# redmod-team/SympGPR

Measured on AMD Instinct MI355X. Metric: Gram-build GB/s + Cholesky fp64 TFLOP/s at N=65536 d=2; |alpha-alpha_ref|/|alpha_ref|, higher is better.
Workload: dtype f64

## Files before the change

### include/sympgpr_probe.h

```cpp
#ifndef SYMPGPR_PROBE_H
#define SYMPGPR_PROBE_H
#include <stddef.h>
#ifdef __cplusplus
extern "C" {
#endif

int sgpr_probe_mfma_f64(int waves_per_simd, int iters, double *tflops);
int sgpr_probe_hbm_write(size_t bytes, int reps, double *gbs);
int sgpr_probe_mfma_clock(int nacc, int waves_per_simd, int iters, double *out3);
int sgpr_probe_gemm(int m, int n, int k, int lower, double *out4);
int sgpr_probe_gemm_debug(int bits);
int sgpr_probe_leaf(double *out8);
int sgpr_probe_lat(double *out8);
int sgpr_probe_xcc(int nblocks, int *host_out);
int sgpr_probe_cumask(const unsigned *mask_words, int nwords, int nblocks, int *host_out);

int sgpr_probe_generated_eval(int family, int which, int m, const double *xa, const double *ya,
                              const double *xb, const double *yb, const double *l, int nl, double *out);

int sgpr_probe_queue_plan(int n, int nworkers, int *starts_out, int max_starts, unsigned *tasks_out, int max_tasks,
                          int *counts);
int sgpr_probe_queue_plan_partial(int n, int nworkers, int nq, int *starts_out, int max_starts, unsigned *tasks_out,
                                  int max_tasks, int *counts);
int sgpr_probe_queue_trace_begin(int max_tasks);
int sgpr_probe_queue_trace_end(unsigned long long *out, int max_tasks);
int sgpr_probe_queue_trace_clear(void);
int sgpr_probe_queue_postmortem(int always);
int sgpr_probe_queue_force_giveup(int on);
int sgpr_probe_tune(const char *name, double value);
int sgpr_probe_strassen_plan(int m, int n, int k, int lower, long smin, long kslab, long scratch_doubles, long long *out,
                             int max_records, int *count);
int sgpr_probe_gemm_strassen_dev(int m, int n, int k, double alpha, const double *A, size_t lda, const double *B, size_t ldb,
                                 double beta, double *C, size_t ldc, int lower, void *stream);
int sgpr_probe_gemm_nt2_dev(int m, int n, int k, double alpha, const double *A, size_t lda, const double *B, size_t ldb,
                            double beta, double *C, size_t ldc, double alpha2, double *C2, size_t ldc2, void *stream);
int sgpr_probe_strassen2_plan(int m, int n, int k, int lower, long smin, long kslab, long smin2, long kslab2, long scratch_doubles,
                              long long *out, int max_records, int *count);
int sgpr_probe_gemm_nt4_dev(int m, int n, int k, const double *A, size_t lda, const double *B, size_t ldb, double beta, int count,
                            double *const *C, const size_t *ldc, const double *alpha, void *stream);
int sgpr_probe_strassen_rec_plan(int m, int n, int k, int lower, long scratch_doubles, long cfg_out[5], long long *out,
                                 int max_records, int *count);
int sgpr_probe_strassen_rec_scratch(int n, unsigned long long out[2]);
int sgpr_probe_gemm_strassen_rec_dev(int m, int n, int k, double alpha, const double *A, size_t lda, const double *B, size_t ldb,
                                     double beta, double *C, size_t ldc, int lower, void *stream);
int sgpr_probe_strassen_schedule(int m, int n, int k, int lower, long capacity_doubles, long long info[12], long long *out,
                                 int max_records, int *count);
int sgpr_probe_batch_layout(int path, int mode, int d, int reg, int nbatch, int n_pts, int nhyp, unsigned long long out[24]);
int sgpr_probe_batch_layout_nd_loo(int path, int mode, int d, int nbatch, int n_pts, int nhyp, unsigned long long out[24]);
int sgpr_probe_batch_layout_loograd_mid(int d, int reg, int nbatch, int n_pts, int nhyp, unsigned long long out[32]);
unsigned sgpr_probe_map_calls(void);
int sgpr_probe_map_team(int ntest, int n0);

int sgpr_probe_trsm_piece(int ticket, int cap, int strips, int out[5]);
int sgpr_probe_trsm_counts(int strips, int cap, unsigned long long out[2]);

int sgpr_probe_census(int na, int threads_a, int lds_a, int spin_a, const unsigned *mask_a, int nwords_a,
                      int nb, int threads_b, int lds_b, int spin_b, const unsigned *mask_b, int nwords_b,
                      unsigned long long *host_out);

int sgpr_probe_strassen_top_plan(int m, int n, int k, int lower, long scratch_doubles, long long *out, int max_records, int *count);
int sgpr_probe_strassen_cfg_plan(int m, int n, int k, int lower, const long cfg[5], long long *out, int max_records, int *count);
int sgpr_probe_strassen_top_scratch(int n, unsigned long long out[2]);
int sgpr_probe_gemm_strassen_top_dev(int m, int n, int k, double alpha, const double *A, size_t lda, const double *B, size_t ldb,
                                     double beta, double *C, size_t ldc, int lower, void *stream);

#ifdef __cplusplus
}
#endif
#endif
```

### sympgpr_amd/_lib.py

```python
import ctypes as C
import os

import numpy as np

FAMILIES = {"A": 0, "B": 1, "C": 2, "D": 3, "USER": 4}
K_KERN, K_DXDX0, K_DYDY0, K_DXDY0 = 0, 1, 2, 3
K_DLX, K_DLY = 4, 8
K_DX, K_DY, K_DX0, K_DY0, K_DXDX0DY0, K_DYDY0DY0, K_DXDY0DY0 = 16, 17, 18, 19, 20, 21, 22
G_QQ, G_PQ, G_QP, G_PP, G_ALL, G_LOWER, G_OCML, G_DLX, G_DLY = 1, 2, 4, 8, 15, 16, 32, 64, 128
FIT_LOWER_ONLY, FIT_REG, FIT_BLOCK_QQ, FIT_BLOCK_PP = 1, 4, 8, 16
MAP_WRAP_Q, MAP_WRAP_P, MAP_EXPLICIT, MAP_LOSS_NEGP = 1, 2, 4, 8
E_ARG, E_NODEVICE, E_HIP, E_NOMEM, E_STATE = -1, -2, -3, -4, -5
LOO_LPD, LOO_PRESS = 0, 1

ABI_VERSION = 5
_dp = C.POINTER(C.c_double)
_vp = C.c_void_p


class SympGPRError(RuntimeError):
    code = None
    detail = ""


class NoDeviceError(SympGPRError):
    pass


def lib_path():
    return os.path.join(os.path.dirname(os.path.abspath(__file__)), "lib", "libsympgpr_hip.so")


SIGNATURES = {
    "sgpr_abi_version": (C.c_int, []),
    "sgpr_last_error": (C.c_char_p, []),
    "sgpr_device_count": (C.c_int, []),
    "sgpr_set_device": (C.c_int, [C.c_int]),
    "sgpr_build_k_host": (C.c_int, [C.c_int, C.c_int, C.c_int, _dp, _dp, _dp, _dp, _dp, C.c_int, _dp, C.c_size_t]),
    "sgpr_buildkreg_host": (C.c_int, [C.c_int, C.c_int, C.c_int, _dp, _dp, _dp, _dp, _dp, C.c_int, _dp, C.c_size_t]),
    "sgpr_build_dk_host": (C.c_int, [C.c_int, C.c_int, C.c_int, C.c_int, _dp, _dp, _dp, _dp, _dp, C.c_int, _dp,
                                     C.c_size_t]),
    "sgpr_build_dkreg_host": (C.c_int, [C.c_int, C.c_int, C.c_int, C.c_int, _dp, _dp, _dp, _dp, _dp, C.c_int, _dp,
                                        C.c_size_t]),
    "sgpr_build_k_nd_host": (C.c_int, [C.c_int, C.c_int, C.c_int, C.c_int, _dp, C.c_size_t, _dp, C.c_size_t, _dp,
                                       C.c_int, _dp, C.c_size_t]),
    "sgpr_kernel_eval_host": (C.c_int, [C.c_int, C.c_int, C.c_int, _dp, _dp, _dp, _dp, _dp, C.c_int, _dp]),
    "sgpr_potrf_host": (C.c_int, [C.c_int, _dp, C.c_size_t]),
    "sgpr_potrs_host": (C.c_int, [C.c_int, _dp, C.c_size_t, _dp, C.c_size_t, C.c_int]),
    "sgpr_fit_create": (C.c_int, [C.c_int, C.c_int, _dp, _dp, _dp, _dp, C.c_int, C.c_double, C.c_uint, _vp,
                                  C.POINTER(_vp)]),
    "sgpr_fit_create_nd": (C.c_int, [C.c_int, C.c_int, C.c_int, _dp, C.c_size_t, _dp, _dp, C.c_int, C.c_double,
                                     C.c_uint, _vp, C.POINTER(_vp)]),
    "sgpr_fit_set_hyp": (C.c_int, [_vp, _dp, C.c_int, C.c_double]),
    "sgpr_fit_set_targets": (C.c_int, [_vp, _dp]),
    "sgpr_fit_build": (C.c_int, [_vp]),
    "sgpr_fit_factor": (C.c_int, [_vp]),
    "sgpr_fit_solve": (C.c_int, [_vp]),
    "sgpr_fit_run": (C.c_int, [_vp]),
    "sgpr_fit_alpha": (C.c_int, [_vp, _dp]),
    "sgpr_fit_nll": (C.c_int, [_vp, _dp]),
    "sgpr_fit_ldiag": (C.c_int, [_vp, _dp]),
    "sgpr_fit_get_matrix": (C.c_int, [_vp, _dp, C.c_size_t]),
    "sgpr_fit_solve_rhs": (C.c_int, [_vp, _dp, C.c_size_t, C.c_int]),
    "sgpr_fit_solve_rhs_dev": (C.c_int, [C.c_void_p, C.c_void_p, C.c_size_t, C.c_int]),
    "sgpr_fit_predict_rows": (C.c_int, [_vp, C.c_int, _dp, _dp, _dp, _dp]),
    "sgpr_fit_nll_grad": (C.c_int, [_vp, _dp]),
    "sgpr_fit_nll_grad_terms": (C.c_int, [_vp, _dp]),
    "sgpr_fit_eig": (C.c_int, [_vp, _dp, _dp]),
    "sgpr_syev_host": (C.c_int, [C.c_int, _dp, C.c_size_t, _dp]),
    "sgpr_fit_inverse": (C.c_int, [_vp, _dp, C.c_size_t]),
    "sgpr_fit_predict_nd": (C.c_int, [_vp, C.c_int, _dp, C.c_size_t, _dp]),
    "sgpr_fit_predict_cov": (C.c_int, [_vp, C.c_int, _dp, C.c_size_t, _dp, _dp]),
    "sgpr_fit_predict_genfun": (C.c_int, [_vp, C.c_int, _dp, C.c_size_t, _dp, _dp, _dp]),
    "sgpr_fit_nll_grad_full": (C.c_int, [_vp, _dp, C.c_int]),
    "sgpr_fit_loo": (C.c_int, [_vp, _dp, _dp, _dp, _dp]),
    "sgpr_fit_loo_grad": (C.c_int, [_vp, C.c_int, _dp, _dp, C.c_int]),
    "sgpr_fit_stage_ms": (C.c_int, [_vp, _dp, _dp, _dp]),
    "sgpr_fit_cond_estimate": (C.c_int, [_vp, C.c_int, _dp]),
    "sgpr_fit_trim": (C.c_int, [_vp]),
    "sgpr_fit_solve_rhs_ms": (C.c_int, [_vp, _dp]),
    "sgpr_potrf_info_dev": (C.c_int, [C.c_int, _vp]),
    "sgpr_trim": (C.c_int, []),
    "sgpr_fit_device_ptrs": (C.c_int, [_vp, C.POINTER(_vp), C.POINTER(C.c_size_t), C.POINTER(_vp)]),
    "sgpr_fit_destroy": (C.c_int, [_vp]),
    "sgpr_gram_pairs_dev": (C.c_int, [C.c_int, C.c_int, C.c_int, _vp, _vp, _vp, _vp, _dp, C.c_int, _vp, _vp, _vp,
                                      _vp, C.c_size_t, C.c_long, C.c_double, C.c_uint, _vp]),
    "sgpr_gram_nd_dev": (C.c_int, [C.c_int, C.c_int, C.c_int, C.c_int, _vp, C.c_size_t, _vp, C.c_size_t, _dp, C.c_int,
                                   _vp, C.c_size_t, C.c_size_t, C.c_size_t, C.c_long, C.c_double, _vp]),
    "sgpr_gram_reg_dev": (C.c_int, [C.c_int, C.c_int, C.c_int, _vp, _vp, _vp, _vp, _dp, C.c_int, _vp, C.c_size_t,
                                    C.c_long, C.c_double, _vp]),
    "sgpr_gram_nd_sel_dev": (C.c_int, [C.c_int, C.c_int, C.c_int, C.c_int, _vp, C.c_size_t, _vp, C.c_size_t, _dp, C.c_int,
                                       _vp, C.c_size_t, C.POINTER(C.c_long), C.POINTER(C.c_long), _vp]),
    "sgpr_potrf_workspace": (C.c_size_t, [C.c_int]),
    "sgpr_potrf_inverses_bytes": (C.c_size_t, [C.c_int]),
    "sgpr_release_device_streams": (C.c_int, [C.c_int]),
    "sgpr_family_has_p": (C.c_int, [C.c_int]),
    "sgpr_potrf_dev": (C.c_int, [C.c_int, _vp, C.c_size_t, _vp, C.c_size_t, _vp, _vp]),
    "sgpr_trsm_rlt_dev": (C.c_int, [C.c_int, C.c_int, _vp, C.c_size_t, _vp, C.c_size_t, _vp, _vp]),
    "sgpr_gemm_nt_dev": (C.c_int, [C.c_int, C.c_int, C.c_int, C.c_double, _vp, C.c_size_t, _vp, C.c_size_t,
                                   C.c_double, _vp, C.c_size_t, C.c_int, C.c_long, _vp]),
    "sgpr_profile_begin": (C.c_int, []),
    "sgpr_profile_end": (C.c_int, [_dp]),
    "sgpr_profile_launches": (C.c_int, [_dp, C.c_int]),
    "sgpr_gemm_nt_bc_dev": (C.c_int, [C.c_int, C.c_int, C.c_int, C.c_double, _vp, C.c_size_t, _vp, C.c_size_t,
                                      C.c_double, _vp, C.c_size_t, C.c_int, C.c_int, C.c_int, C.c_int, C.c_int, _vp]),
    "sgpr_trsv_dev": (C.c_int, [C.c_int, _vp, C.c_size_t, _vp, _vp, C.c_int, _vp]),
    "sgpr_gemv_sub_dev": (C.c_int, [C.c_int, C.c_int, C.c_int, _vp, C.c_size_t, _vp, _vp, _vp]),
    "sgpr_gemm_nn_dev": (C.c_int, [C.c_int, C.c_int, C.c_int, C.c_double, _vp, C.c_size_t, _vp, C.c_size_t, C.c_double, _vp,
                                   C.c_size_t, _vp]),
    "sgpr_trsm_rl_dev": (C.c_int, [C.c_int, C.c_int, _vp, C.c_size_t, _vp, C.c_size_t, _vp, _vp]),
    "sgpr_copy_blocks_dev": (C.c_int, [C.c_int, C.c_int, C.c_int, _vp, C.c_size_t, C.c_size_t, _vp, C.c_size_t, C.c_size_t, _vp]),
    "sgpr_predict_rows_dev": (C.c_int, [C.c_int, C.c_int, _vp, _vp, C.c_int, _vp, _vp, _dp, C.c_int, _vp, _vp, _vp,
                                        _vp]),
    "sgpr_predict_nd_dev": (C.c_int, [C.c_int, C.c_int, C.c_int, _vp, C.c_size_t, C.c_int, _vp, C.c_size_t, _dp, C.c_int,
                                      _vp, _vp, _vp]),
    "sgpr_predict_reg_dev": (C.c_int, [C.c_int, C.c_int, _vp, _vp, C.c_int, _vp, _vp, _dp, C.c_int, _vp, _vp, _vp]),
    "sgpr_applymap_host": (C.c_int, [C.c_int, C.c_int, C.c_int, C.c_int, _dp, C.c_int, C.c_int, _dp, _dp, _dp, _dp,
                                     C.c_int, C.c_int, _dp, _dp, _dp, _dp, _dp, _dp, _dp, _dp]),
    "sgpr_applymap_sections_host": (C.c_int, [C.c_int, C.c_int, C.c_int, C.c_int, C.c_int, C.c_int, _dp, C.c_int, C.c_int, _dp, _dp,
                                              _dp, _dp, C.c_int, C.c_int, _dp, _dp, _dp, _dp, _dp, _dp, _dp, _dp]),
    "sgpr_applymap_sections_tangent_host": (C.c_int, [C.c_int, C.c_int, C.c_int, C.c_int, C.c_int, C.c_int, _dp, C.c_int, C.c_int,
                                                      _dp, _dp, _dp, _dp, C.c_int, C.c_int, _dp, _dp, _dp, _dp, _dp, _dp, _dp, _dp,
                                                      _dp, _dp, _dp]),
    "sgpr_applymap_sections_inverse_host": (C.c_int, [C.c_int, C.c_int, C.c_int, C.c_int, C.c_int, C.c_int, _dp, C.c_int, C.c_int,
                                                      _dp, _dp, _dp, _dp, _dp, _dp, _dp, C.POINTER(C.c_int)]),
    "sgpr_fit_applymap_nd": (C.c_int, [_vp, C.c_int, C.c_int, C.c_int, _dp, C.c_size_t, _dp, C.c_size_t, _dp, _dp,
                                       C.POINTER(C.c_int)]),
    "sgpr_applymap_nd_host": (C.c_int, [C.c_int, C.c_int, C.c_int, C.c_int, C.c_int, _dp, C.c_int, C.c_int, _dp, C.c_size_t,
                                        _dp, _dp, C.c_size_t, _dp, C.c_size_t, _dp, _dp, C.POINTER(C.c_int)]),
    "sgpr_fit_applymap_nd_tangent": (C.c_int, [_vp, C.c_int, C.c_int, C.c_int, _dp, C.c_size_t, _dp, C.c_size_t, _dp, _dp,
                                               C.POINTER(C.c_int), _dp, _dp, _dp]),
    "sgpr_applymap_nd_tangent_host": (C.c_int, [C.c_int, C.c_int, C.c_int, C.c_int, C.c_int, _dp, C.c_int, C.c_int, _dp,
                                                C.c_size_t, _dp, _dp, C.c_size_t, _dp, C.c_size_t, _dp, _dp, C.POINTER(C.c_int),
                                                _dp, _dp, _dp]),
    "sgpr_fit_applymap_nd_inverse": (C.c_int, [_vp, C.c_int, C.c_int, C.c_int, _dp, C.c_size_t, _dp, C.c_size_t, _dp, _dp,
                                               C.POINTER(C.c_int)]),
    "sgpr_applymap_nd_inverse_host": (C.c_int, [C.c_int, C.c_int, C.c_int, C.c_int, C.c_int, _dp, C.c_int, C.c_int, _dp,
                                                C.c_size_t, _dp, _dp, C.c_size_t, _dp, C.c_size_t, _dp, _dp, C.POINTER(C.c_int)]),
    "sgpr_fit_periodic_nd": (C.c_int, [_vp, C.c_int, C.c_int, C.c_int, C.POINTER(C.c_int), _dp, C.c_size_t, _dp, C.c_size_t,
                                       C.c_double, C.c_int, _dp, _dp, C.POINTER(C.c_int), _dp, _dp, _dp]),
    "sgpr_periodic_nd_host": (C.c_int, [C.c_int, C.c_int, C.c_int, C.c_int, C.c_int, _dp, C.c_int, C.c_int, _dp, C.c_size_t,
                                        _dp, C.POINTER(C.c_int), _dp, C.c_size_t, _dp, C.c_size_t, C.c_double, C.c_int, _dp, _dp,
                                        C.POINTER(C.c_int), _dp, _dp, _dp]),
    "sgpr_potrs_vec_dev": (C.c_int, [C.c_int, _vp, C.c_size_t, _vp, _vp, _vp]),
    "sgpr_solve_status_dev": (C.c_int, [C.c_int, _vp, C.c_size_t, _vp, _vp]),
    "sgpr_fit_batch_max_order": (C.c_int, []),
    "sgpr_fit_batch": (C.c_int, [C.c_int, C.c_int, C.c_int, _dp, _dp, _dp, _dp, C.c_int, _dp, C.c_uint, _dp, _dp,
                                 C.POINTER(C.c_int)]),
    "sgpr_fit_batch_nd": (C.c_int, [C.c_int, C.c_int, C.c_int, C.c_int, _dp, _dp, _dp, C.c_int, _dp, C.c_uint, _dp, _dp,
                                    C.POINTER(C.c_int)]),
    "sgpr_fit_batch_nd_grad": (C.c_int, [C.c_int, C.c_int, C.c_int, C.c_int, _dp, _dp, _dp, C.c_int, _dp, C.c_uint, _dp, _dp, _dp,
                                         C.POINTER(C.c_int)]),
    "sgpr_fit_batch_nd_loo": (C.c_int, [C.c_int, C.c_int, C.c_int, C.c_int, _dp, _dp, _dp, C.c_int, _dp, C.c_uint, _dp, _dp, _dp,
                                        C.POINTER(C.c_int)]),
    "sgpr_fit_batch_nd_loo_grad": (C.c_int, [C.c_int, C.c_int, C.c_int, C.c_int, _dp, _dp, _dp, C.c_int, _dp, C.c_uint, C.c_int, _dp,
                                             _dp, _dp, _dp, C.POINTER(C.c_int)]),
    "sgpr_fit_batch_grad": (C.c_int, [C.c_int, C.c_int, C.c_int, _dp, _dp, _dp, _dp, C.c_int, _dp, C.c_uint, _dp, _dp, _dp,
                                      C.POINTER(C.c_int)]),
    "sgpr_fit_batch_grad_mid": (C.c_int, [C.c_int, C.c_int, C.c_int, _dp, _dp, _dp, _dp, C.c_int, _dp, C.c_uint, _dp, _dp, _dp,
                                          C.POINTER(C.c_int)]),
    "sgpr_fit_batch_loo": (C.c_int, [C.c_int, C.c_int, C.c_int, _dp, _dp, _dp, _dp, C.c_int, _dp, C.c_uint, _dp, _dp, _dp,
                                     C.POINTER(C.c_int)]),
    "sgpr_fit_batch_loo_grad": (C.c_int, [C.c_int, C.c_int, C.c_int, _dp, _dp, _dp, _dp, C.c_int, _dp, C.c_uint, C.c_int, _dp,
                                          _dp, _dp, _dp, C.POINTER(C.c_int)]),
    "sgpr_fit_batch_loo_grad_mid": (C.c_int, [C.c_int, C.c_int, C.c_int, _dp, _dp, _dp, _dp, C.c_int, _dp, C.c_uint, C.c_int, _dp,
                                              _dp, _dp, _dp, C.POINTER(C.c_int)]),
    "sgpr_fit_batch_nd_loo_grad_mid": (C.c_int, [C.c_int, C.c_int, C.c_int, C.c_int, _dp, _dp, _dp, C.c_int, _dp, C.c_uint, C.c_int,
                                                 _dp, _dp, _dp, _dp, C.POINTER(C.c_int)]),
}

PROBE_SIGNATURES = {
    "sgpr_probe_mfma_f64": (C.c_int, [C.c_int, C.c_int, _dp]),
    "sgpr_probe_mfma_clock": (C.c_int, [C.c_int, C.c_int, C.c_int, _dp]),
    "sgpr_probe_gemm": (C.c_int, [C.c_int, C.c_int, C.c_int, C.c_int, _dp]),
    "sgpr_probe_gemm_debug": (C.c_int, [C.c_int]),
    "sgpr_probe_leaf": (C.c_int, [_dp]),
    "sgpr_probe_lat": (C.c_int, [_dp]),
    "sgpr_probe_cumask": (C.c_int, [C.POINTER(C.c_uint), C.c_int, C.c_int, C.POINTER(C.c_int)]),
    "sgpr_probe_xcc": (C.c_int, [C.c_int, C.POINTER(C.c_int)]),
    "sgpr_probe_hbm_write": (C.c_int, [C.c_size_t, C.c_int, _dp]),
    "sgpr_probe_generated_eval": (C.c_int, [C.c_int, C.c_int, C.c_int, _dp, _dp, _dp, _dp, _dp, C.c_int, _dp]),
    "sgpr_probe_queue_plan": (C.c_int, [C.c_int, C.c_int, C.POINTER(C.c_int), C.c_int, C.POINTER(C.c_uint), C.c_int,
                                        C.POINTER(C.c_int)]),
    "sgpr_probe_queue_plan_partial": (C.c_int, [C.c_int, C.c_int, C.c_int, C.POINTER(C.c_int), C.c_int, C.POINTER(C.c_uint),
                                                C.c_int, C.POINTER(C.c_int)]),
    "sgpr_probe_queue_trace_begin": (C.c_int, [C.c_int]),
    "sgpr_probe_queue_trace_end": (C.c_int, [C.POINTER(C.c_ulonglong), C.c_int]),
    "sgpr_probe_queue_postmortem": (C.c_int, [C.c_int]),
    "sgpr_probe_queue_force_giveup": (C.c_int, [C.c_int]),
    "sgpr_probe_tune": (C.c_int, [C.c_char_p, C.c_double]),
    "sgpr_probe_map_calls": (C.c_uint, []),
    "sgpr_probe_map_team": (C.c_int, [C.c_int, C.c_int]),
    "sgpr_probe_trsm_piece": (C.c_int, [C.c_int, C.c_int, C.c_int, C.POINTER(C.c_int)]),
    "sgpr_probe_trsm_counts": (C.c_int, [C.c_int, C.c_int, C.POINTER(C.c_ulonglong)]),
    "sgpr_probe_queue_trace_clear": (C.c_int, []),
    "sgpr_probe_strassen_plan": (C.c_int, [C.c_int, C.c_int, C.c_int, C.c_int, C.c_long, C.c_long, C.c_long,
                                           C.POINTER(C.c_longlong), C.c_int, C.POINTER(C.c_int)]),
    "sgpr_probe_gemm_strassen_dev": (C.c_int, [C.c_int, C.c_int, C.c_int, C.c_double, C.c_void_p, C.c_size_t, C.c_void_p, C.c_size_t,
                                               C.c_double, C.c_void_p, C.c_size_t, C.c_int, C.c_void_p]),
    "sgpr_probe_gemm_nt2_dev": (C.c_int, [C.c_int, C.c_int, C.c_int, C.c_double, C.c_void_p, C.c_size_t, C.c_void_p, C.c_size_t,
                                          C.c_double, C.c_void_p, C.c_size_t, C.c_double, C.c_void_p, C.c_size_t, C.c_void_p]),
    "sgpr_probe_strassen2_plan": (C.c_int, [C.c_int, C.c_int, C.c_int, C.c_int, C.c_long, C.c_long, C.c_long, C.c_long, C.c_long,
                                            C.POINTER(C.c_longlong), C.c_int, C.POINTER(C.c_int)]),
    "sgpr_probe_strassen_rec_plan": (C.c_int, [C.c_int, C.c_int, C.c_int, C.c_int, C.c_long, C.POINTER(C.c_long),
                                               C.POINTER(C.c_longlong), C.c_int, C.POINTER(C.c_int)]),
    "sgpr_probe_strassen_rec_scratch": (C.c_int, [C.c_int, C.POINTER(C.c_ulonglong)]),
    "sgpr_probe_strassen_schedule": (C.c_int, [C.c_int, C.c_int, C.c_int, C.c_int, C.c_long, C.POINTER(C.c_longlong),
                                               C.POINTER(C.c_longlong), C.c_int, C.POINTER(C.c_int)]),
    "sgpr_probe_gemm_strassen_rec_dev": (C.c_int, [C.c_int, C.c_int, C.c_int, C.c_double, C.c_void_p, C.c_size_t, C.c_void_p, C.c_size_t,
                                                   C.c_double, C.c_void_p, C.c_size_t, C.c_int, C.c_void_p]),
    "sgpr_probe_strassen_top_plan": (C.c_int, [C.c_int, C.c_int, C.c_int, C.c_int, C.c_long, C.POINTER(C.c_longlong), C.c_int,
                                               C.POINTER(C.c_int)]),
    "sgpr_probe_strassen_cfg_plan": (C.c_int, [C.c_int, C.c_int, C.c_int, C.c_int, C.POINTER(C.c_long), C.POINTER(C.c_longlong), C.c_int,
                                               C.POINTER(C.c_int)]),
    "sgpr_probe_strassen_top_scratch": (C.c_int, [C.c_int, C.POINTER(C.c_ulonglong)]),
    "sgpr_probe_gemm_strassen_top_dev": (C.c_int, [C.c_int, C.c_int, C.c_int, C.c_double, C.c_void_p, C.c_size_t, C.c_void_p, C.c_size_t,
                                                   C.c_double, C.c_void_p, C.c_size_t, C.c_int, C.c_void_p]),
    "sgpr_probe_gemm_nt4_dev": (C.c_int, [C.c_int, C.c_int, C.c_int, C.c_void_p, C.c_size_t, C.c_void_p, C.c_size_t, C.c_double, C.c_int,
                                          C.c_void_p, C.POINTER(C.c_size_t), C.POINTER(C.c_double), C.c_void_p]),
    "sgpr_probe_batch_layout": (C.c_int, [C.c_int, C.c_int, C.c_int, C.c_int, C.c_int, C.c_int, C.c_int,
                                          C.POINTER(C.c_ulonglong)]),
    "sgpr_probe_batch_layout_nd_loo": (C.c_int, [C.c_int, C.c_int, C.c_int, C.c_int, C.c_int, C.c_int, C.POINTER(C.c_ulonglong)]),
    "sgpr_probe_batch_layout_loograd_mid": (C.c_int, [C.c_int, C.c_int, C.c_int, C.c_int, C.c_int, C.POINTER(C.c_ulonglong)]),
    "sgpr_probe_census": (C.c_int, [C.c_int, C.c_int, C.c_int, C.c_int, C.POINTER(C.c_uint), C.c_int,
                                    C.c_int, C.c_int, C.c_int, C.c_int, C.POINTER(C.c_uint), C.c_int,
                                    C.POINTER(C.c_ulonglong)]),
}

_LIB = None
_PROBE = None


def load_library():
    global _LIB
    if _LIB is not None:
        return _LIB
    path = lib_path()
    if os.environ.get("SYMPGPR_NO_TORCH_PRELOAD") != "1":
        try:
            import torch
        except ImportError:
            pass
    if not os.path.exists(path):
        raise SympGPRError("%s is missing: run `python -c 'import __graft_entry__ as g; g.build()'` "
                           "(or make -C sympgpr_amd/csrc); there is no CPU fallback" % path)
    lib = C.CDLL(path)
    for name, (res, args) in SIGNATURES.items():
        fn = getattr(lib, name)
        fn.restype = res
        fn.argtypes = args
    if lib.sgpr_abi_version() != ABI_VERSION:
        raise SympGPRError("ABI version mismatch: %s is version %d, this package binds version %d -- rebuild it "
                           "(make -C sympgpr_amd/csrc)" % (path, lib.sgpr_abi_version(), ABI_VERSION))
    _LIB = lib
    import atexit
    atexit.register(_release_streams_at_exit)
    return lib


def _release_streams_at_exit():
    lib = _LIB
    if lib is None:
        return
    try:
        for dev in range(max(0, lib.sgpr_device_count())):
            lib.sgpr_release_device_streams(dev)
    except Exception:
        pass


def load_probe_library():
    global _PROBE
    if _PROBE is not None:
        return _PROBE
    load_library()
    path = os.path.join(os.path.dirname(lib_path()), "libsympgpr_probe.so")
    if not os.path.exists(path):
        raise SympGPRError("%s is missing: run make -C sympgpr_amd/csrc" % path)
    lib = C.CDLL(path)
    for name, (res, args) in PROBE_SIGNATURES.items():
        fn = getattr(lib, name)
        fn.restype = res
        fn.argtypes = args
    _PROBE = lib
    return lib


def device_count():
    return load_library().sgpr_device_count()


def check(rc, what=""):
    if rc == 0:
        return
    if rc > 0:
        raise np.linalg.LinAlgError("%d-th leading minor of the array is not positive definite" % rc)
    msg = load_library().sgpr_last_error().decode(errors="replace")
    err = (NoDeviceError(msg) if rc == E_NODEVICE else
           SympGPRError("%s failed (%d): %s" % (what or "libsympgpr_hip call", rc, msg)))
    err.code, err.detail = rc, msg
    raise err


def dptr(a):
    return a.ctypes.data_as(_dp)


def f64(a):
    return np.ascontiguousarray(np.asarray(a, dtype=np.float64))


def family_has_p(fam):
    return bool(load_library().sgpr_family_has_p(family_id(fam)))


def family_id(fam):
    if isinstance(fam, str):
        return FAMILIES[fam]
    return int(fam)
```

### sympgpr_amd/csrc/probe.hip

```cpp
#include <algorithm>
#include <cstdlib>
#include <vector>

#include "cholq.h"
#include "common.h"
#include "strassen.h"
#include "../../include/sympgpr_probe.h"
#include "generated/pair_generated.h"
#include "nd_eval.h"

namespace sgpr {
namespace {
typedef double double4_t __attribute__((ext_vector_type(4)));
typedef double double2_t __attribute__((ext_vector_type(2)));

template <int NACC>
__global__ __launch_bounds__(256) void mfma_clock_kernel(int iters, double *out, unsigned long long *stamps)
{
    double4_t acc[NACC];
    const double a = 1.0 + threadIdx.x * 1e-9, b = 1.0 - threadIdx.x * 1e-9;
#pragma unroll
    for (int i = 0; i < NACC; ++i) acc[i] = double4_t{0.0, 0.0, 0.0, 0.0};
    const unsigned long long t0 = __builtin_amdgcn_s_memtime(), r0 = __builtin_amdgcn_s_memrealtime();
    for (int it = 0; it < iters; ++it) {
#pragma unroll
        for (int i = 0; i < NACC; ++i)
            asm volatile("v_mfma_f64_16x16x4_f64 %0, %1, %2, %0" : "+v"(acc[i]) : "v"(a), "v"(b));
    }
    asm volatile("s_nop 15\n\ts_nop 15" ::: "memory");
    double s = 0.0;
#pragma unroll
    for (int i = 0; i < NACC; ++i) s += acc[i][0] + acc[i][1] + acc[i][2] + acc[i][3];
    const unsigned long long t1 = __builtin_amdgcn_s_memtime(), r1 = __builtin_amdgcn_s_memrealtime();
    if (s == 12345.678) out[0] = s;
    if (threadIdx.x == 0) {
        stamps[4 * blockIdx.x + 0] = t0; stamps[4 * blockIdx.x + 1] = t1;
        stamps[4 * blockIdx.x + 2] = r0; stamps[4 * blockIdx.x + 3] = r1;
    }
}

__global__ __launch_bounds__(256) void mfma_probe_kernel(int iters, double *out)
{
    double4_t acc[8];
    const double a = 1.0 + threadIdx.x * 1e-9, b = 1.0 - threadIdx.x * 1e-9;
#pragma unroll
    for (int i = 0; i < 8; ++i) acc[i] = double4_t{0.0, 0.0, 0.0, 0.0};
    for (int it = 0; it < iters; ++it) {
#pragma unroll
        for (int i = 0; i < 8; ++i) acc[i] = __builtin_amdgcn_mfma_f64_16x16x4f64(a, b, acc[i], 0, 0, 0);
    }
    double s = 0.0;
#pragma unroll
    for (int i = 0; i < 8; ++i) s += acc[i][0] + acc[i][1] + acc[i][2] + acc[i][3];
    if (s == 12345.678) out[0] = s;
}

__global__ __launch_bounds__(256) void write_probe_kernel(double2_t *dst, size_t n2)
{
    const size_t stride = (size_t)gridDim.x * blockDim.x;
    const double2_t v{1.0, 2.0};
    for (size_t i = (size_t)blockIdx.x * blockDim.x + threadIdx.x; i < n2; i += stride) dst[i] = v;
}
}
}

using namespace sgpr;

extern "C" int sgpr_probe_mfma_f64(int waves_per_simd, int iters, double *tflops)
{
    double *d = nullptr;
    SGPR_HIP(hipMalloc((void **)&d, 64));
    hipEvent_t a, b;
    SGPR_HIP(hipEventCreate(&a));
    SGPR_HIP(hipEventCreate(&b));
    const int blocks = 256 * waves_per_simd;
    hipLaunchKernelGGL(mfma_probe_kernel, dim3(blocks), dim3(256), 0, nullptr, iters / 10 + 1, d);
    SGPR_HIP(hipEventRecord(a, nullptr));
    hipLaunchKernelGGL(mfma_probe_kernel, dim3(blocks), dim3(256), 0, nullptr, iters, d);
    SGPR_HIP(hipEventRecord(b, nullptr));
    SGPR_HIP(hipEventSynchronize(b));
    float ms = 0.f;
    SGPR_HIP(hipEventElapsedTime(&ms, a, b));
    *tflops = (double)blocks * 4 * iters * 8 * 2048.0 / (ms * 1e-3) / 1e12;
    (void)hipEventDestroy(a); (void)hipEventDestroy(b); (void)hipFree(d);
    return 0;
}

extern "C" int sgpr_probe_mfma_clock(int nacc, int waves_per_simd, int iters, double *out3)
{
    const int blocks = 256 * waves_per_simd;
    double *d = nullptr;
    unsigned long long *st = nullptr;
    SGPR_HIP(hipMalloc((void **)&d, 64));
    SGPR_HIP(hipMalloc((void **)&st, sizeof(unsigned long long) * 4 * blocks));
    hipEvent_t a, b;
    SGPR_HIP(hipEventCreate(&a));
    SGPR_HIP(hipEventCreate(&b));
    auto launch = [&](int it) {
        if (nacc == 4) hipLaunchKernelGGL((mfma_clock_kernel<4>), dim3(blocks), dim3(256), 0, nullptr, it, d, st);
        else if (nacc == 16) hipLaunchKernelGGL((mfma_clock_kernel<16>), dim3(blocks), dim3(256), 0, nullptr, it, d, st);
        else hipLaunchKernelGGL((mfma_clock_kernel<8>), dim3(blocks), dim3(256), 0, nullptr, it, d, st);
    };
    if (nacc != 4 && nacc != 16) nacc = 8;
    launch(iters);
    SGPR_HIP(hipEventRecord(a, nullptr));
    launch(iters);
    SGPR_HIP(hipEventRecord(b, nullptr));
    SGPR_HIP(hipEventSynchronize(b));
    float ms = 0.f;
    SGPR_HIP(hipEventElapsedTime(&ms, a, b));
    std::vector<unsigned long long> h(4 * (size_t)blocks);
    SGPR_HIP(hipMemcpy(h.data(), st, h.size() * sizeof(unsigned long long), hipMemcpyDeviceToHost));
    std::vector<double> cyc(blocks), ghz(blocks);
    for (int i = 0; i < blocks; ++i) {
        const double dc = (double)(h[4 * i + 1] - h[4 * i]), dr = (double)(h[4 * i + 3] - h[4 * i + 2]);
        cyc[i] = dc / ((double)iters * nacc) / waves_per_simd;
        ghz[i] = dr > 0 ? dc / (dr * 10.0) : 0.0;
    }
    std::sort(cyc.begin(), cyc.end());
    std::sort(ghz.begin(), ghz.end());
    out3[0] = (double)blocks * 4 * iters * nacc * 2048.0 / (ms * 1e-3) / 1e12;
    out3[1] = cyc[blocks / 2];
    out3[2] = ghz[blocks / 2];
    (void)hipEventDestroy(a); (void)hipEventDestroy(b); (void)hipFree(d); (void)hipFree(st);
    return 0;
}

extern "C" int sgpr_probe_hbm_write(size_t bytes, int reps, double *gbs)
{
    double *d = nullptr;
    SGPR_HIP(hipMalloc((void **)&d, bytes));
    hipEvent_t a, b;
    SGPR_HIP(hipEventCreate(&a));
    SGPR_HIP(hipEventCreate(&b));
    hipLaunchKernelGGL(write_probe_kernel, dim3(2048), dim3(256), 0, nullptr, (double2_t *)d, bytes / 16);
    SGPR_HIP(hipEventRecord(a, nullptr));
    for (int r = 0; r < reps; ++r)
        hipLaunchKernelGGL(write_probe_kernel, dim3(2048), dim3(256), 0, nullptr, (double2_t *)d, bytes / 16);
    SGPR_HIP(hipEventRecord(b, nullptr));
    SGPR_HIP(hipEventSynchronize(b));
    float ms = 0.f;
    SGPR_HIP(hipEventElapsedTime(&ms, a, b));
    *gbs = (double)bytes * reps / (ms * 1e-3) / 1e9;
    (void)hipEventDestroy(a); (void)hipEventDestroy(b); (void)hipFree(d);
    return 0;
}

static thread_local int t_probe_dbg = 0;
extern "C" int sgpr_probe_gemm_debug(int bits) { t_probe_dbg = bits; return 0; }

extern "C" int sgpr_probe_gemm(int m, int n, int k, int lower, double *out4)
{
    double *A = nullptr, *B = nullptr, *Cm = nullptr;
    unsigned long long *st = nullptr;
    const char *pe = getenv("SGPR_PROBE_PAD");
    const size_t pad = pe ? (size_t)atoi(pe) : 0;
    const size_t lda = (size_t)m + pad, ldb = (size_t)n + pad, ldc = (size_t)m + pad;
    SGPR_HIP(hipMalloc((void **)&A, sizeof(double) * lda * k));
    SGPR_HIP(hipMalloc((void **)&B, sizeof(double) * ldb * k));
    SGPR_HIP(hipMalloc((void **)&Cm, sizeof(double) * ldc * n));
    const size_t nwg = (size_t)((m + 127) / 128 + 8) * ((n + 127) / 128 + 8);
    SGPR_HIP(hipMalloc((void **)&st, sizeof(unsigned long long) * 4 * nwg));
    SGPR_HIP(hipMemset(st, 0, sizeof(unsigned long long) * 4 * nwg));
    KConst kc;
    const double hyp[3] = {0.7, 0.9, 1.0};
    make_kconst(SGPR_FAM_C, hyp, 3, &kc);
    std::vector<double> h((size_t)std::max(m, n) + k);
    for (size_t i = 0; i < h.size(); ++i) h[i] = 0.37 * (double)((i * 2654435761u) % 1000) / 100.0;
    double *pts = nullptr;
    SGPR_HIP(hipMalloc((void **)&pts, sizeof(double) * h.size()));
    SGPR_HIP(hipMemcpy(pts, h.data(), sizeof(double) * h.size(), hipMemcpyHostToDevice));
    gram_reg(SGPR_FAM_C, m, k, pts, pts, pts + 3, pts + 5, kc, A, lda, 0, 0.0, nullptr);
    gram_reg(SGPR_FAM_C, n, k, pts, pts + 1, pts + 2, pts + 7, kc, B, ldb, 0, 0.0, nullptr);
    SGPR_HIP(hipMemset(Cm, 0, sizeof(double) * ldc * n));
    hipEvent_t a, b;
    SGPR_HIP(hipEventCreate(&a));
    SGPR_HIP(hipEventCreate(&b));
    const char *be = getenv("SGPR_PROBE_BETA");
    const double beta = be ? atof(be) : 1.0;
    int rc = gemm_nt_diag(m, n, k, -1.0, A, lda, B, ldb, beta, Cm, ldc, lower, nullptr, t_probe_dbg, nullptr);
    if (rc) return rc;
    SGPR_HIP(hipEventRecord(a, nullptr));
    rc = gemm_nt_diag(m, n, k, -1.0, A, lda, B, ldb, beta, Cm, ldc, lower, st, t_probe_dbg, nullptr);
    SGPR_HIP(hipEventRecord(b, nullptr));
    if (rc) return rc;
    SGPR_HIP(hipEventSynchronize(b));
    float ms = 0.f;
    SGPR_HIP(hipEventElapsedTime(&ms, a, b));
    std::vector<unsigned long long> hs(4 * nwg);
    SGPR_HIP(hipMemcpy(hs.data(), st, hs.size() * sizeof(unsigned long long), hipMemcpyDeviceToHost));
    std::vector<double> cyc, ghz;
    for (size_t i = 0; i < nwg; ++i) {
        if (hs[4 * i + 1] == 0) continue;
        const double dc = (double)(hs[4 * i + 1] - hs[4 * i]), dr = (double)(hs[4 * i + 3] - hs[4 * i + 2]);
        cyc.push_back(dc);
        if (dr > 0) ghz.push_back(dc / (dr * 10.0));
    }
    std::sort(cyc.begin(), cyc.end());
    std::sort(ghz.begin(), ghz.end());
    double flop = 2.0 * m * n * (double)k;
    if (lower) flop *= 0.5;
    out4[0] = flop / (ms * 1e-3) / 1e12;
    out4[1] = cyc.empty() ? 0 : cyc[cyc.size() / 2];
    out4[2] = ghz.empty() ? 0 : ghz[ghz.size() / 2];
    out4[3] = (k + 15) / 16;
    (void)hipFree(A); (void)hipFree(B); (void)hipFree(Cm); (void)hipFree(st); (void)hipFree(pts);
    (void)hipEventDestroy(a); (void)hipEventDestroy(b);
    return 0;
}


namespace sgpr { namespace {
template <int V>
__global__ __launch_bounds__(256) void lat_probe_kernel(double *io, unsigned long long *cyc)
{
    __shared__ double sh[64];
    __shared__ double big[16 * 130];
    const int lane = threadIdx.x & 63, l15 = lane & 15, l4 = lane >> 4;
    if (threadIdx.x >= 64) return;
    double mneg[16];
#pragma unroll
    for (int j = 0; j < 16; ++j) mneg[j] = (l4 == (j & 3) && l15 > j) ? -1.0 : 0.0;
    double4_t D, X;
#pragma unroll
    for (int r = 0; r < 4; ++r) { D[r] = (4 * r + l4 == l15) ? 4.0 + 0.01 * l15 : 1.0 / (2.0 + l15 + 4 * r + l4); X[r] = (4 * r + l4 == l15) ? 1.0 : 0.0; }
    double rl = io[0], acc = io[1];
    auto bcast = [&](double v, int ln) {
        const unsigned lo = __builtin_amdgcn_readlane((int)__double2loint(v), ln);
        const unsigned hi = __builtin_amdgcn_readlane((int)__double2hiint(v), ln);
        return __hiloint2double((int)hi, (int)lo);
    };
    auto nr = [&](double d) {
        double r = __builtin_amdgcn_rsq(d);
        r = r * __builtin_fma(-0.5 * d * r, r, 1.5);
        r = r * __builtin_fma(-0.5 * d * r, r, 1.5);
        return r;
    };
    unsigned long long t0, t1;
    asm volatile("s_memtime %0\n\ts_waitcnt lgkmcnt(0)" : "=s"(t0), "+v"(rl), "+v"(acc), "+v"(D), "+v"(X) : : "memory");
#pragma unroll
    for (int j = 0; j < 16; ++j) {
        const int rj = j >> 2;
        if (V == 0) {
            const double v = D[rj] * rl;
            D = __builtin_amdgcn_mfma_f64_16x16x4f64(v, v, D, 0, 0, 0);
        } else if (V == 1) {
            const double v = D[rj] * rl, x = X[rj] * rl;
            D = __builtin_amdgcn_mfma_f64_16x16x4f64(v, v, D, 0, 0, 0);
            X = __builtin_amdgcn_mfma_f64_16x16x4f64(v, x, X, 0, 0, 0);
        } else if (V == 2) {
            const double a = bcast(acc, (j + 1) & 63), b = bcast(rl, (j + 17) & 63);
            rl = nr(__builtin_fma(-b, b, a + 5.0));
            acc += rl;
        } else if (V == 3) {
            rl = __builtin_amdgcn_rsq(rl + 1.0);
        } else if (V == 4) {
#pragma unroll
            for (int q = 0; q < 8; ++q) rl = __builtin_fma(rl, acc, 0.5);
        } else if (V == 5) {
            rl = bcast(rl, (j + 1) & 63) + acc;
        } else if (V == 6) {
            sh[lane] = rl;
            rl = sh[(lane + 1) & 63] + 1.0;
        } else if (V >= 8) {
            const int g = j & 3;
            const double v = D[rj] * rl;
            const double x = X[rj] * rl;
            double rn = 0.0;
            if (j + 1 < 16) {
                const double dnext = bcast(D[(j + 1) >> 2], (j + 1) + 16 * ((j + 1) & 3));
                const double lnext = bcast(v, (j + 1) + 16 * g);
                rn = nr(__builtin_fma(-lnext, lnext, dnext));
            }
            if (V == 8 || V == 9) {
                if (l4 == g) big[j * 130 + l15] = v;
                sh[j] = rl;
            }
            const double nv = v * mneg[j];
            D = __builtin_amdgcn_mfma_f64_16x16x4f64(nv, v, D, 0, 0, 0);
            if (V == 8 || V == 10) X = __builtin_amdgcn_mfma_f64_16x16x4f64(nv, x, X, 0, 0, 0);
            rl = rn;
        } else if (V == 7) {
            const double v = D[rj] * rl;
            D = __builtin_amdgcn_mfma_f64_16x16x4f64(v, v, D, 0, 0, 0);
            rl = bcast(D[0], 0) * 1e-3;
        }
    }
    double ssum = rl + acc + D[0] + D[1] + D[2] + D[3] + X[0] + X[1] + X[2] + X[3];
    asm volatile("s_nop 0\n\ts_memtime %0\n\ts_waitcnt lgkmcnt(0)" : "=s"(t1), "+v"(ssum) : : "memory");
    if (lane == 0) cyc[V] = t1 - t0;
    if (ssum == 12345.678) io[2] = ssum + big[lane] + sh[lane];
}
} }

extern "C" int sgpr_probe_lat(double *out8 )
{
    double *io = nullptr;
    unsigned long long *cyc = nullptr;
    SGPR_HIP(hipMalloc((void **)&io, 64));
    SGPR_HIP(hipMalloc((void **)&cyc, 128));
    const double h[3] = {0.49, 1.25, 0.0};
    SGPR_HIP(hipMemcpy(io, h, sizeof(h), hipMemcpyHostToDevice));
    for (int rep = 0; rep < 2; ++rep) {
        hipLaunchKernelGGL((sgpr::lat_probe_kernel<0>), dim3(1), dim3(256), 0, 0, io, cyc);
        hipLaunchKernelGGL((sgpr::lat_probe_kernel<1>), dim3(1), dim3(256), 0, 0, io, cyc);
        hipLaunchKernelGGL((sgpr::lat_probe_kernel<2>), dim3(1), dim3(256), 0, 0, io, cyc);
        hipLaunchKernelGGL((sgpr::lat_probe_kernel<3>), dim3(1), dim3(256), 0, 0, io, cyc);
        hipLaunchKernelGGL((sgpr::lat_probe_kernel<4>), dim3(1), dim3(256), 0, 0, io, cyc);
        hipLaunchKernelGGL((sgpr::lat_probe_kernel<5>), dim3(1), dim3(256), 0, 0, io, cyc);
        hipLaunchKernelGGL((sgpr::lat_probe_kernel<6>), dim3(1), dim3(256), 0, 0, io, cyc);
        hipLaunchKernelGGL((sgpr::lat_probe_kernel<7>), dim3(1), dim3(256), 0, 0, io, cyc);
        hipLaunchKernelGGL((sgpr::lat_probe_kernel<8>), dim3(1), dim3(256), 0, 0, io, cyc);
        hipLaunchKernelGGL((sgpr::lat_probe_kernel<9>), dim3(1), dim3(256), 0, 0, io, cyc);
        hipLaunchKernelGGL((sgpr::lat_probe_kernel<10>), dim3(1), dim3(256), 0, 0, io, cyc);
        hipLaunchKernelGGL((sgpr::lat_probe_kernel<11>), dim3(1), dim3(256), 0, 0, io, cyc);
        SGPR_HIP(hipDeviceSynchronize());
    }
    unsigned long long hs[12];
    SGPR_HIP(hipMemcpy(hs, cyc, 96, hipMemcpyDeviceToHost));
    for (int i = 0; i < 12; ++i) out8[i] = (double)hs[i] / 16.0;
    (void)hipFree(io); (void)hipFree(cyc);
    return 0;
}

extern "C" int sgpr_probe_leaf(double *out8)
{
    const int n = LEAF;
    std::vector<double> h((size_t)n * n, 0.0);
    for (int i = 0; i < n; ++i)
        for (int j = 0; j <= i; ++j) h[i + (size_t)j * n] = (i == j) ? 4.0 + 0.01 * i : 1.0 / (1.0 + i + j);
    double *A = nullptr, *inv = nullptr;
    int *info = nullptr;
    unsigned long long *st = nullptr;
    SGPR_HIP(hipMalloc((void **)&A, sizeof(double) * n * n));
    SGPR_HIP(hipMalloc((void **)&inv, sizeof(double) * n * n));
    SGPR_HIP(hipMalloc((void **)&info, 16));
    SGPR_HIP(hipMalloc((void **)&st, 64));
    SGPR_HIP(hipMemset(info, 0, 16));
    for (int rep = 0; rep < 2; ++rep) {
        SGPR_HIP(hipMemcpy(A, h.data(), sizeof(double) * n * n, hipMemcpyHostToDevice));
        int rc = leaf_probe(A, n, inv, info, st, nullptr);
        if (rc) return rc;
        SGPR_HIP(hipDeviceSynchronize());
    }
    unsigned long long hs[8];
    SGPR_HIP(hipMemcpy(hs, st, 64, hipMemcpyDeviceToHost));
    for (int i = 0; i < 8; ++i) out8[i] = (double)hs[i];
    (void)hipFree(A); (void)hipFree(inv); (void)hipFree(info); (void)hipFree(st);
    return 0;
}

namespace sgpr { namespace {
__global__ __launch_bounds__(512) void xcc_probe_kernel(int *out)
{
    const int x = __builtin_amdgcn_s_getreg(20 | (0 << 6) | (3 << 11));
    if (threadIdx.x == 0) out[blockIdx.x] = x;
    unsigned long long t0 = __builtin_amdgcn_s_memtime();
    while (__builtin_amdgcn_s_memtime() - t0 < 20000) {}
}
} }
extern "C" int sgpr_probe_xcc(int nblocks, int *host_out)
{
    int *d = nullptr;
    SGPR_HIP(hipMalloc((void **)&d, sizeof(int) * nblocks));
    hipLaunchKernelGGL(sgpr::xcc_probe_kernel, dim3(nblocks), dim3(512), 0, nullptr, d);
    SGPR_HIP(hipMemcpy(host_out, d, sizeof(int) * nblocks, hipMemcpyDeviceToHost));
    (void)hipFree(d);
    return 0;
}

namespace sgpr { namespace {
__global__ __launch_bounds__(512) void cumask_probe_kernel(int *out)
{
    const int x = __builtin_amdgcn_s_getreg(20 | (0 << 6) | (3 << 11));
    const int hw = __builtin_amdgcn_s_getreg(4 | (0 << 6) | (31 << 11));
    if (threadIdx.x == 0) { out[2 * blockIdx.x] = x; out[2 * blockIdx.x + 1] = hw; }
    unsigned long long t0 = __builtin_amdgcn_s_memtime();
    while (__builtin_amdgcn_s_memtime() - t0 < 200000) {}
}
} }
extern "C" int sgpr_probe_cumask(const unsigned *mask_words, int nwords, int nblocks, int *host_out)
{
    hipStream_t st = nullptr;
    SGPR_HIP(hipExtStreamCreateWithCUMask(&st, (uint32_t)nwords, mask_words));
    int *d = nullptr;
    SGPR_HIP(hipMalloc((void **)&d, sizeof(int) * 2 * nblocks));
    hipLaunchKernelGGL(sgpr::cumask_probe_kernel, dim3(nblocks), dim3(512), 0, st, d);
    SGPR_HIP(hipStreamSynchronize(st));
    SGPR_HIP(hipMemcpy(host_out, d, sizeof(int) * 2 * nblocks, hipMemcpyDeviceToHost));
    (void)hipFree(d);
    (void)hipStreamDestroy(st);
    return 0;
}


namespace sgpr {
template <int FAM>
__global__ void generated_eval_kernel(int which, int m, const double *xa, const double *ya, const double *xb,
                                      const double *yb, double lx, double ly, double p, double *out)
{
    const int i = blockIdx.x * blockDim.x + threadIdx.x;
    if (i >= m) return;
    double o[4];
    const int dl = which >> 2;
    if (dl == 0)      gen::pair<FAM>(xa[i], ya[i], xb[i], yb[i], lx, ly, p, o);
    else if (dl == 1) gen::pair_dlx<FAM>(xa[i], ya[i], xb[i], yb[i], lx, ly, p, o);
    else              gen::pair_dly<FAM>(xa[i], ya[i], xb[i], yb[i], lx, ly, p, o);
    out[i] = o[which & 3];
}
}

extern "C" int sgpr_probe_generated_eval(int family, int which, int m, const double *xa, const double *ya,
                                         const double *xb, const double *yb, const double *l, int nl, double *out)
{
    using namespace sgpr;
    if (m <= 0) return 0;
    if (which < 0 || which > 11 || !l || nl < 2 || (family == SGPR_FAM_D && nl < 3)) { set_error("generated_eval: bad arguments"); return SGPR_E_ARG; }
    double *d[5] = {};
    const double *h[4] = {xa, ya, xb, yb};
    for (int k = 0; k < 5; ++k) SGPR_HIP(hipMalloc((void **)&d[k], sizeof(double) * m));
    for (int k = 0; k < 4; ++k) SGPR_HIP(hipMemcpy(d[k], h[k], sizeof(double) * m, hipMemcpyHostToDevice));
    const double p = family == SGPR_FAM_D ? l[2] : 0.0;
    const dim3 grid((m + 255) / 256);
    switch (family) {
    case SGPR_FAM_A: hipLaunchKernelGGL(generated_eval_kernel<SGPR_FAM_A>, grid, dim3(256), 0, nullptr, which, m, d[0], d[1], d[2], d[3], l[0], l[1], p, d[4]); break;
    case SGPR_FAM_B: hipLaunchKernelGGL(generated_eval_kernel<SGPR_FAM_B>, grid, dim3(256), 0, nullptr, which, m, d[0], d[1], d[2], d[3], l[0], l[1], p, d[4]); break;
    case SGPR_FAM_C: hipLaunchKernelGGL(generated_eval_kernel<SGPR_FAM_C>, grid, dim3(256), 0, nullptr, which, m, d[0], d[1], d[2], d[3], l[0], l[1], p, d[4]); break;
    case SGPR_FAM_D: hipLaunchKernelGGL(generated_eval_kernel<SGPR_FAM_D>, grid, dim3(256), 0, nullptr, which, m, d[0], d[1], d[2], d[3], l[0], l[1], p, d[4]); break;
    default: set_error("unknown kernel family"); return SGPR_E_ARG;
    }
    SGPR_CHECK_LAUNCH();
    SGPR_HIP(hipMemcpy(out, d[4], sizeof(double) * m, hipMemcpyDeviceToHost));
    for (int k = 0; k < 5; ++k) (void)hipFree(d[k]);
    return 0;
}

extern "C" int sgpr_probe_queue_plan(int n, int nworkers, int *starts_out, int max_starts, unsigned *tasks_out,
                                     int max_tasks, int *counts)
{
    cholq::Plan p;
    const int rc = cholq::build_plan(n, cholq::default_starts(n), nworkers, p);
    if (rc) return rc;
    counts[0] = p.nblk;
    counts[1] = (int)(p.tasks.size() / 2);
    counts[2] = (int)p.model_us;
    for (int k = 0; k <= p.nblk && k < max_starts; ++k) starts_out[k] = p.starts[k];
    for (size_t t = 0; t < p.tasks.size() && (int)(t / 2) < max_tasks; ++t) tasks_out[t] = p.tasks[t];
    return 0;
}

extern "C" int sgpr_probe_queue_plan_partial(int n, int nworkers, int nq, int *starts_out, int max_starts, unsigned *tasks_out,
                                             int max_tasks, int *counts)
{
    cholq::Plan p;
    const std::vector<int> st = cholq::default_starts(n);
    const int rc = cholq::build_plan(n, st, nworkers, p, nq < 0 ? cholq::default_nq(n, st) : nq);
    if (rc) return rc;
    counts[0] = p.nblk;
    counts[1] = (int)(p.tasks.size() / 2);
    counts[2] = (int)p.model_us;
    counts[3] = p.nq;
    for (int k = 0; k <= p.nblk && k < max_starts; ++k) starts_out[k] = p.starts[k];
    for (size_t t = 0; t < p.tasks.size() && (int)(t / 2) < max_tasks; ++t) tasks_out[t] = p.tasks[t];
    return 0;
}

static unsigned long long *g_qtrace = nullptr;
static int g_qtrace_cap = 0;
extern "C" int sgpr_probe_queue_trace_begin(int max_tasks)
{
    if (g_qtrace) { cholq::set_trace(nullptr, 0); (void)hipFree(g_qtrace); g_qtrace = nullptr; }
    SGPR_HIP(hipMalloc((void **)&g_qtrace, sizeof(unsigned long long) * cholq::trace_words((size_t)max_tasks)));
    SGPR_HIP(hipMemset(g_qtrace, 0, sizeof(unsigned long long) * cholq::trace_words((size_t)max_tasks)));
    g_qtrace_cap = max_tasks;
    cholq::set_trace(g_qtrace, (size_t)max_tasks);
    return max_tasks;
}
extern "C" int sgpr_probe_queue_trace_clear()
{
    if (!g_qtrace) return 0;
    SGPR_HIP(hipMemset(g_qtrace, 0, sizeof(unsigned long long) * cholq::trace_words((size_t)g_qtrace_cap)));
    return 0;
}
extern "C" int sgpr_probe_queue_trace_end(unsigned long long *out, int max_tasks)
{
    if (!g_qtrace) return 0;
    SGPR_HIP(hipDeviceSynchronize());
    cholq::set_trace(nullptr, 0);
    if (max_tasks < g_qtrace_cap) { set_error("queue_trace_end: buffer smaller than the capacity given to _begin"); return SGPR_E_ARG; }
    const size_t words = cholq::trace_words((size_t)g_qtrace_cap);
    SGPR_HIP(hipMemcpy(out, g_qtrace, sizeof(unsigned long long) * words, hipMemcpyDeviceToHost));
    (void)hipFree(g_qtrace);
    g_qtrace = nullptr;
    return (int)words;
}

extern "C" int sgpr_probe_queue_postmortem(int always) { return cholq::postmortem(always != 0); }
extern "C" int sgpr_probe_queue_force_giveup(int on) { cholq::force_giveup(on); return 0; }
extern "C" int sgpr_probe_tune(const char *name, double value)
{
    if (!name) { set_error("probe_tune: null name"); return SGPR_E_ARG; }
    tune_set(name, value);
    return 0;
}

extern "C" int sgpr_probe_strassen_plan(int m, int n, int k, int lower, long smin, long kslab, long scratch_doubles, long long *out,
                                        int max_records, int *count)
{
    if (!count || scratch_doubles < 0) { set_error("probe_strassen_plan: bad arguments"); return SGPR_E_ARG; }
    std::vector<long long> plan;
    const int rc = strassen_plan(m, n, k, lower, smin, kslab, (size_t)scratch_doubles, plan);
    if (rc) return rc;
    *count = (int)(plan.size() / STRASSEN_REC);
    for (size_t i = 0; out && i < plan.size() && (int)(i / STRASSEN_REC) < max_records; ++i) out[i] = plan[i];
    return 0;
}
extern "C" int sgpr_probe_gemm_strassen_dev(int m, int n, int k, double alpha, const double *A, size_t lda, const double *B, size_t ldb,
                                            double beta, double *C, size_t ldc, int lower, void *stream)
{
    return gemm_nt_strassen(m, n, k, alpha, A, lda, B, ldb, beta, C, ldc, lower, static_cast<hipStream_t>(stream));
}
extern "C" int sgpr_probe_gemm_nt2_dev(int m, int n, int k, double alpha, const double *A, size_t lda, const double *B, size_t ldb,
                                       double beta, double *C, size_t ldc, double alpha2, double *C2, size_t ldc2, void *stream)
{
    return gemm_nt_two(m, n, k, alpha, A, lda, B, ldb, beta, C, ldc, alpha2, C2, ldc2, static_cast<hipStream_t>(stream));
}
extern "C" int sgpr_probe_strassen2_plan(int m, int n, int k, int lower, long smin, long kslab, long smin2, long kslab2,
                                         long scratch_doubles, long long *out, int max_records, int *count)
{
    if (!count || scratch_doubles < 0) { set_error("probe_strassen2_plan: bad arguments"); return SGPR_E_ARG; }
    std::vector<long long> plan;
    const int rc = strassen_outer_plan(m, n, k, lower, smin, kslab, smin2, kslab2, (size_t)scratch_doubles, plan);
    if (rc) return rc;
    *count = (int)(plan.size() / STRASSEN_REC);
    for (size_t i = 0; out && i < plan.size() && (int)(i / STRASSEN_REC) < max_records; ++i) out[i] = plan[i];
    return 0;
}
extern "C" int sgpr_probe_strassen_rec_plan(int m, int n, int k, int lower, long scratch_doubles, long cfg_out[5], long long *out,
                                            int max_records, int *count)
{
    if (!count || scratch_doubles < 0) { set_error("probe_strassen_rec_plan: bad arguments"); return SGPR_E_ARG; }
    std::vector<long long> plan;
    const int rc = strassen_rec_plan(m, n, k, lower, cfg_out, (size_t)scratch_doubles, plan);
    if (rc) return rc;
    *count = (int)(plan.size() / STRASSEN_REC);
    for (size_t i = 0; out && i < plan.size() && (int)(i / STRASSEN_REC) < max_records; ++i) out[i] = plan[i];
    return 0;
}
extern "C" int sgpr_probe_strassen_rec_scratch(int n, unsigned long long out[2])
{
    if (n < 0 || !out) { set_error("probe_strassen_rec_scratch: bad arguments"); return SGPR_E_ARG; }
    size_t need[2];
    potrf_strassen_need(n, need);
    out[0] = need[0]; out[1] = need[1];
    return 0;
}
extern "C" int sgpr_probe_strassen_schedule(int m, int n, int k, int lower, long capacity_doubles, long long info[12], long long *out,
                                            int max_records, int *count)
{
    if (!count) { set_error("probe_strassen_schedule: bad arguments"); return SGPR_E_ARG; }
    std::vector<long long> sched;
    const int rc = strassen_schedule(m, n, k, lower, (long long)capacity_doubles, info, sched);
    if (rc) return rc;
    *count = (int)(sched.size() / SCHED_REC);
    for (size_t i = 0; out && i < sched.size() && (int)(i / SCHED_REC) < max_records; ++i) out[i] = sched[i];
    return 0;
}
extern "C" int sgpr_probe_gemm_strassen_rec_dev(int m, int n, int k, double alpha, const double *A, size_t lda, const double *B, size_t ldb,
                                                double beta, double *C, size_t ldc, int lower, void *stream)
{
    return gemm_nt_strassen_rec(m, n, k, alpha, A, lda, B, ldb, beta, C, ldc, lower, static_cast<hipStream_t>(stream));
}
extern "C" int sgpr_probe_gemm_nt4_dev(int m, int n, int k, const double *A, size_t lda, const double *B, size_t ldb, double beta,
                                       int count, double *const *C, const size_t *ldc, const double *alpha, void *stream)
{
    return gemm_nt_multi(m, n, k, A, lda, B, ldb, beta, count, C, ldc, alpha, static_cast<hipStream_t>(stream));
}
extern "C" int sgpr_probe_strassen_top_plan(int m, int n, int k, int lower, long scratch_doubles, long long *out, int max_records, int *count)
{
    if (!count || scratch_doubles < 0) { set_error("probe_strassen_top_plan: bad arguments"); return SGPR_E_ARG; }
    std::vector<long long> plan;
    const int rc = strassen_top_plan(m, n, k, lower, nullptr, nullptr, (size_t)scratch_doubles, plan);
    if (rc) return rc;
    *count = (int)(plan.size() / STRASSEN_REC);
    for (size_t i = 0; out && i < plan.size() && (int)(i / STRASSEN_REC) < max_records; ++i) out[i] = plan[i];
    return 0;
}
extern "C" int sgpr_probe_strassen_cfg_plan(int m, int n, int k, int lower, const long cfg[5], long long *out, int max_records, int *count)
{
    if (!count) { set_error("probe_strassen_cfg_plan: bad arguments"); return SGPR_E_ARG; }
    std::vector<long long> plan;
    const int rc = strassen_cfg_plan(m, n, k, lower, cfg, plan);
    if (rc) return rc;
    *count = (int)(plan.size() / STRASSEN_REC);
    for (size_t i = 0; out && i < plan.size() && (int)(i / STRASSEN_REC) < max_records; ++i) out[i] = plan[i];
    return 0;
}
extern "C" int sgpr_probe_strassen_top_scratch(int n, unsigned long long out[2])
{
    if (n < 0 || !out) { set_error("probe_strassen_top_scratch: bad arguments"); return SGPR_E_ARG; }
    out[0] = potrf_strassen_top_need(n);
    out[1] = 2 * out[0];
    return 0;
}
extern "C" int sgpr_probe_gemm_strassen_top_dev(int m, int n, int k, double alpha, const double *A, size_t lda, const double *B, size_t ldb,
                                                double beta, double *C, size_t ldc, int lower, void *stream)
{
    return strassen_top_gemm(m, n, k, alpha, A, lda, B, ldb, beta, C, ldc, lower, nullptr, nullptr, static_cast<hipStream_t>(stream));
}
static int probe_batch_layout(const char *entry, bool nd_loo, int path, int mode, int d, int reg, int nbatch, int n_pts, int nhyp,
                              unsigned long long out[24])
{
    const long n = d ? 2L * d * n_pts : reg ? (long)n_pts : 2L * n_pts;
    if (path < 0 || path > 1 || mode < 0 || mode > 3 || (path && mode == 3) || d < 0 || d > 3 || (d && (reg || (mode > 1 && !nd_loo))) ||
        nbatch < 1 || n_pts < 1 || nhyp < 1 || (path ? n <= 256 || n > 2048 : n > 256) || !out) {
        set_error(std::string(entry) + ": bad arguments");
        return SGPR_E_ARG;
    }
    const BatchLayout l = batch_layout(path, mode, d, reg, nbatch, n_pts, nhyp);
    const size_t v[24] = {(size_t)l.chunk, l.nacc, l.o_x, l.o_y, l.o_z, l.o_kc, l.o_no, l.in_bytes, l.o_al, l.o_nll, l.o_info, l.out_bytes,
                          l.o_A, l.o_inv, l.o_fl, l.o_fl2, l.o_r, l.o_pub, l.o_st, l.o_part, l.scr_bytes,
                          sizeof(KConst), sizeof(nd::NdConst), l.flag_bytes};
    for (int i = 0; i < 24; ++i) out[i] = v[i];
    return 0;
}
extern "C" int sgpr_probe_batch_layout(int path, int mode, int d, int reg, int nbatch, int n_pts, int nhyp, unsigned long long out[24])
{
    return probe_batch_layout("probe_batch_layout", false, path, mode, d, reg, nbatch, n_pts, nhyp, out);
}
extern "C" int sgpr_probe_batch_layout_nd_loo(int path, int mode, int d, int nbatch, int n_pts, int nhyp, unsigned long long out[24])
{
    if (d < 1 || (mode != 2 && mode != 3)) {
        set_error("probe_batch_layout_nd_loo: d is 1 .. 3 and mode 2 (loo) or 3 (loo gradient)");
        return SGPR_E_ARG;
    }
    return probe_batch_layout("probe_batch_layout_nd_loo", true, path, mode, d, 0, nbatch, n_pts, nhyp, out);
}
extern "C" int sgpr_probe_batch_layout_loograd_mid(int d, int reg, int nbatch, int n_pts, int nhyp, unsigned long long out[32])
{
    const long n = d ? 2L * d * n_pts : reg ? (long)n_pts : 2L * n_pts;
    if (d < 0 || d > 3 || reg < 0 || reg > 1 || (d && reg) || nbatch < 1 || n_pts < 1 || nhyp < 1 || n <= 256 || n > 2048 || !out) {
        set_error("probe_batch_layout_loograd_mid: bad arguments (256 < order <= 2048)");
        return SGPR_E_ARG;
    }
    const BatchLayout l = batch_layout(1, 3, d, reg, nbatch, n_pts, nhyp);
    const size_t v[32] = {(size_t)l.chunk, l.nacc, l.o_x, l.o_y, l.o_z, l.o_kc, l.o_no, l.in_bytes, l.o_al, l.o_nll, l.o_info, l.out_bytes,
                          l.o_A, l.o_inv, l.o_fl, l.o_fl2, l.o_r, l.o_pub, l.o_st, l.o_part, l.scr_bytes,
                          sizeof(KConst), sizeof(nd::NdConst), l.flag_bytes, l.o_lpart, l.o_wt, l.o_v, l.o_beta, l.o_zero, (size_t)l.npad, 3, 0};
    for (int i = 0; i < 32; ++i) out[i] = v[i];
    return 0;
}
extern "C" unsigned sgpr_probe_map_calls(void) { return applymap_last_calls(); }
extern "C" int sgpr_probe_map_team(int ntest, int n0) { return applymap_team(ntest, n0); }
extern "C" int sgpr_probe_trsm_piece(int ticket, int cap, int strips, int out[5]) { if (ticket < 0 || cap < 1 || strips < 0 || !out) return SGPR_E_ARG; trsm_piece_of(ticket, cap, strips, out); return 0; }
extern "C" int sgpr_probe_trsm_counts(int strips, int cap, unsigned long long out[2])
{
    if (strips < 0 || cap < 1 || !out) return SGPR_E_ARG;
    size_t c[2];
    trsm_piece_counts(strips, cap, c);
    out[0] = c[0]; out[1] = c[1];
    return 0;
}

namespace sgpr { namespace {
__global__ void census_kernel(unsigned long long *out, int spin_us)
{
    extern __shared__ double dyn[];
    const unsigned long long t0 = __builtin_amdgcn_s_memrealtime();
    if (threadIdx.x == 0) {
        dyn[0] = 1.0;
        out[4 * blockIdx.x + 0] = (unsigned long long)__builtin_amdgcn_s_getreg(20 | (0 << 6) | (3 << 11));
        out[4 * blockIdx.x + 1] = (unsigned long long)__builtin_amdgcn_s_getreg(4 | (0 << 6) | (31 << 11));
        out[4 * blockIdx.x + 2] = t0;
    }
    while (__builtin_amdgcn_s_memrealtime() - t0 < (unsigned long long)spin_us * 100ull) __builtin_amdgcn_s_sleep(32);
    if (threadIdx.x == 0) out[4 * blockIdx.x + 3] = __builtin_amdgcn_s_memrealtime();
}
} }
extern "C" int sgpr_probe_census(int na, int threads_a, int lds_a, int spin_a, const unsigned *mask_a, int nwords_a,
                                 int nb, int threads_b, int lds_b, int spin_b, const unsigned *mask_b, int nwords_b,
                                 unsigned long long *host_out)
{
    hipStream_t sa = nullptr, sb = nullptr;
    if (nwords_a > 0) SGPR_HIP(hipExtStreamCreateWithCUMask(&sa, (uint32_t)nwords_a, mask_a));
    else              SGPR_HIP(hipStreamCreateWithFlags(&sa, hipStreamNonBlocking));
    if (nwords_b > 0) SGPR_HIP(hipExtStreamCreateWithCUMask(&sb, (uint32_t)nwords_b, mask_b));
    else {
        int lo = 0, hi = 0;
        SGPR_HIP(hipDeviceGetStreamPriorityRange(&lo, &hi));
        SGPR_HIP(hipStreamCreateWithPriority(&sb, hipStreamNonBlocking, hi));
    }
    unsigned long long *d = nullptr;
    const size_t words = 4 * (size_t)(na + nb);
    SGPR_HIP(hipMalloc((void **)&d, sizeof(unsigned long long) * words));
    SGPR_HIP(hipMemset(d, 0, sizeof(unsigned long long) * words));
    SGPR_HIP(hipFuncSetAttribute((const void *)sgpr::census_kernel, hipFuncAttributeMaxDynamicSharedMemorySize, 160 * 1024));
    SGPR_HIP(hipDeviceSynchronize());
    hipLaunchKernelGGL(sgpr::census_kernel, dim3(na), dim3(threads_a), lds_a, sa, d, spin_a);
    SGPR_CHECK_LAUNCH();
    hipLaunchKernelGGL(sgpr::census_kernel, dim3(nb), dim3(threads_b), lds_b, sb, d + 4 * (size_t)na, spin_b);
    SGPR_CHECK_LAUNCH();
    SGPR_HIP(hipStreamSynchronize(sa));
    SGPR_HIP(hipStreamSynchronize(sb));
    SGPR_HIP(hipMemcpy(host_out, d, sizeof(unsigned long long) * words, hipMemcpyDeviceToHost));
    (void)hipFree(d);
    (void)hipStreamDestroy(sa);
    (void)hipStreamDestroy(sb);
    return 0;
}
```

### sympgpr_amd/csrc/strassen.h

```cpp
#pragma once
#include <algorithm>
#include <cstddef>
#include <string>
#include <vector>

#include "../../include/sympgpr_hip.h"

namespace sgpr {

void set_error(const std::string &msg);
double tune(const char *name, double dflt);

constexpr int STRASSEN_REC = 16;
enum { PLAN_SUM = 1, PLAN_PROD = 2, PLAN_CLASSIC = 3 };
int strassen_plan(int m, int n, int k, int lower, long smin, long kslab, size_t scratch_doubles, std::vector<long long> &out);

enum { PLAN2_SUM = 4, PLAN2_PROD = 5 };
int strassen_outer_plan(int m, int n, int k, int lower, long smin, long kslab, long smin2, long kslab2, size_t scratch_doubles,
                   std::vector<long long> &out);
struct StrassenCfg { long smin = -1, kslab = -1, smin2 = -1, kslab2 = -1, smin_under = -1; };
template <typename T> void cfg_to_words(const StrassenCfg &c, T *w)
{
    w[0] = (T)c.smin; w[1] = (T)c.kslab; w[2] = (T)c.smin2; w[3] = (T)c.kslab2; w[4] = (T)c.smin_under;
}
template <typename T> StrassenCfg cfg_of_words(const T *w)
{
    StrassenCfg c;
    c.smin = (long)w[0]; c.kslab = (long)w[1]; c.smin2 = (long)w[2]; c.kslab2 = (long)w[3]; c.smin_under = (long)w[4];
    return c;
}
inline bool bad_extents(int m, int n, int k, int lower) { return m < 0 || n < 0 || k < 0 || (lower && m != n); }
size_t strassen_scratch_doubles_cfg(int m, int n, int k, int lower, int levels, const StrassenCfg &cfg);
struct StrassenRec { bool on = false; long smin_gemm = 0, smin_syrk = 0, smin2_gemm = 0, smin2_syrk = 0, kslab = 0, kslab2 = 0, kslab2_short = 0; };
StrassenRec strassen_rec_values();
StrassenCfg strassen_rec_cfg(const StrassenRec &v, int k, int lower);
int strassen_rec_plan(int m, int n, int k, int lower, long cfg_out[5], size_t scratch_doubles, std::vector<long long> &out);

constexpr int SCHED_REC = 32;
int strassen_schedule(int m, int n, int k, int lower, long long cap_doubles, long long info[12], std::vector<long long> &out);

enum { PLAN3_SUM = 6, PLAN3_ZERO = 7, PLAN3_PROD = 8, PLAN3_ACC = 9, PLAN3_PASS = 10 };
struct StrassenTop { long smin3 = 0, kslab3 = 0, kslab3_short = 0; };
StrassenTop strassen_top_values();
int strassen_top_plan(int m, int n, int k, int lower, const StrassenRec *v, const StrassenTop *t, size_t scratch_doubles,
                      std::vector<long long> &out);
int strassen_cfg_plan(int m, int n, int k, int lower, const long cfg[5], std::vector<long long> &out);
size_t strassen_top_scratch_doubles(int m, int n, int k, int lower, const StrassenRec &v, const StrassenTop &t);

void potrf_strassen_need(int n, size_t out[2]);
size_t potrf_strassen_top_need(int n);

namespace splan {
struct PlanCfg {
    long smin;
    long kslab;
    size_t scratch;
};
struct Plan2Cfg {
    PlanCfg in;
    long smin2;
    long kslab2;
    size_t scratch;
    long smin_under = -1;
};
struct Need2 { size_t v[4] = {0, 0, 0, 0}; size_t inner() const { return v[0] + v[1]; } size_t total() const { return v[0] + v[1] + v[2] + v[3]; } };
struct SchedCfg {
    int nbuf[4] = {1, 1, 1, 1};
    size_t off[4][2] = {};
    int nstreams = 1;
};
struct Need3 { size_t v[3] = {0, 0, 0}; size_t total() const { return v[0] + v[1] + v[2]; } };

int strassen_levels();
bool outer_noscratch();
Plan2Cfg cfg2_of(const StrassenCfg &cfg, size_t scratch_doubles);
PlanCfg under_of(const Plan2Cfg &c);
void outer_plan_of(int m, int n, int k, int lower, const Plan2Cfg &c, std::vector<long long> &out);
Need2 plan_need(const std::vector<long long> &plan, const Plan2Cfg &c);
SchedCfg sched_cfg_of(const Need2 &nd, size_t cap, bool overlap);
void schedule_of(const std::vector<long long> &plan, const Plan2Cfg &c, const Need2 &nd, const SchedCfg &sc, std::vector<long long> &out);
Need3 top_need(const std::vector<long long> &plan);
int top_buffers_wanted();
}

#ifdef SGPR_HIP_TYPES
int gemm_nt_strassen(int m, int n, int k, double alpha, const double *A, size_t lda, const double *B, size_t ldb, double beta,
                     double *C, size_t ldc, int lower, hipStream_t st);
int gemm_nt_strassen_cfg(int m, int n, int k, double alpha, const double *A, size_t lda, const double *B, size_t ldb, double beta,
                         double *C, size_t ldc, int lower, const StrassenCfg &cfg, hipStream_t st);
int gemm_nt_strassen_rec(int m, int n, int k, double alpha, const double *A, size_t lda, const double *B, size_t ldb, double beta,
                         double *C, size_t ldc, int lower, hipStream_t st);
int strassen_top_gemm(int m, int n, int k, double alpha, const double *A, size_t lda, const double *B, size_t ldb, double beta,
                      double *C, size_t ldc, int lower, const StrassenRec *v, const StrassenTop *t, hipStream_t st);
void strassen_reserve(size_t both, size_t one, hipStream_t st);
void strassen_top_reserve(size_t need, hipStream_t st);
int strassen_trim();
int strassen_sum_streams(hipStream_t caller, int count, hipStream_t *out);
int strassen_top_stream(hipStream_t caller, hipStream_t *out);
#endif

}
```

### sympgpr_amd/csrc/strassen.hip

```cpp
#include <algorithm>
#include <cstdint>
#include <mutex>
#include <vector>

#include "common.h"
#include "gemm_tile.h"
#include "strassen.h"

namespace sgpr {
using namespace splan;

namespace {
using namespace tile;

__global__ __launch_bounds__(256) void block_sum_kernel(int rows, int cols, const double *X, size_t ldx, const double *Y, size_t ldy,
                                                        double sign, double *T)
{
    const int nrc = (rows + 511) / 512, ncg = (cols + 3) / 4;
    const long pieces = (long)nrc * ncg;
    for (long p = blockIdx.x; p < pieces; p += gridDim.x) {
        const int cg = (int)(p / nrc), rc = (int)(p - (long)cg * nrc);
        const int r = rc * 512 + 2 * (int)threadIdx.x;
        if (r >= rows) continue;
        double2_t x[4], y[4];
#pragma unroll
        for (int u = 0; u < 4; ++u) {
            const int c = min(cg * 4 + u, cols - 1);
            x[u] = *reinterpret_cast<const double2_t *>(X + (size_t)r + (size_t)c * ldx);
            y[u] = *reinterpret_cast<const double2_t *>(Y + (size_t)r + (size_t)c * ldy);
        }
#pragma unroll
        for (int u = 0; u < 4; ++u) {
            const int c = cg * 4 + u;
            if (c < cols) *reinterpret_cast<double2_t *>(T + (size_t)r + (size_t)c * (size_t)rows) = x[u] + sign * y[u];
        }
    }
}

__global__ __launch_bounds__(256) void block_acc_kernel(int rows, int cols, const double *T, double *C1, double a1, double *C2, double a2,
                                                        size_t ldc)
{
    const int nrc = (rows + 511) / 512, ncg = (cols + 3) / 4;
    const long pieces = (long)nrc * ncg;
    for (long p = blockIdx.x; p < pieces; p += gridDim.x) {
        const int cg = (int)(p / nrc), rc = (int)(p - (long)cg * nrc);
        const int r = rc * 512 + 2 * (int)threadIdx.x;
        if (r >= rows) continue;
        double2_t t[4], c1[4], c2[4];
#pragma unroll
        for (int u = 0; u < 4; ++u) {
            const int c = min(cg * 4 + u, cols - 1);
            t[u] = *reinterpret_cast<const double2_t *>(T + (size_t)r + (size_t)c * (size_t)rows);
            c1[u] = *reinterpret_cast<const double2_t *>(C1 + (size_t)r + (size_t)c * ldc);
            if (C2) c2[u] = *reinterpret_cast<const double2_t *>(C2 + (size_t)r + (size_t)c * ldc);
        }
#pragma unroll
        for (int u = 0; u < 4; ++u) {
            const int c = cg * 4 + u;
            if (c >= cols) continue;
            *reinterpret_cast<double2_t *>(C1 + (size_t)r + (size_t)c * ldc) = c1[u] + a1 * t[u];
            if (C2) *reinterpret_cast<double2_t *>(C2 + (size_t)r + (size_t)c * ldc) = c2[u] + a2 * t[u];
        }
    }
}

constexpr long SUM_WGS = 2048;
constexpr long SUM_WGS_SIDE = 256;
long side_wgs() { return std::min(65535L, std::max(1L, (long)tune("gemm_strassen_sum_wgs", (double)SUM_WGS_SIDE))); }

int block_sum(int rows, int cols, const double *X, size_t ldx, const double *Y, size_t ldy, double sign, double *T, hipStream_t st, long wgs)
{
    const long pieces = (long)((rows + 511) / 512) * ((cols + 3) / 4);
    hipLaunchKernelGGL(block_sum_kernel, dim3((unsigned)std::min(pieces, wgs)), dim3(256), 0, st, rows, cols, X, ldx, Y, ldy, sign, T);
    SGPR_CHECK_LAUNCH();
    return 0;
}
int block_acc(int rows, int cols, const double *T, double *C1, double a1, double *C2, double a2, size_t ldc, hipStream_t st, long wgs)
{
    const long pieces = (long)((rows + 511) / 512) * ((cols + 3) / 4);
    hipLaunchKernelGGL(block_acc_kernel, dim3((unsigned)std::min(pieces, wgs)), dim3(256), 0, st, rows, cols, T, C1, a1, C2, a2, ldc);
    SGPR_CHECK_LAUNCH();
    return 0;
}

struct Mat { const double *p; size_t ld; };
template <typename T> T *block(T *P, size_t ld, long long row, long long col) { return P + row + (size_t)col * ld; }
int sum_into(const long long *r, Mat A, Mat B, double *T, hipStream_t st, long wgs)
{
    const Mat P = r[1] ? B : A;
    return block_sum((int)r[2], (int)r[3], block(P.p, P.ld, r[4], r[5]), P.ld, block(P.p, P.ld, r[6], r[7]), P.ld, (double)r[8], T, st, wgs);
}
Mat operand_of(const long long *r, int side, Mat P, const double *S)
{
    const long long *o = r + 1 + 3 * side;
    return o[0] ? Mat{S, (size_t)r[7 + side]} : Mat{block(P.p, P.ld, o[1], o[2]), P.ld};
}
struct Dests { double *C1; double a1; double *C2; double a2; };
Dests dests_of(const long long *d, double alpha, double *C, size_t ldc)
{
    return Dests{block(C, ldc, d[0], d[1]), alpha * (double)d[2], d[5] ? block(C, ldc, d[3], d[4]) : nullptr, alpha * (double)d[5]};
}

struct Scratch {
    std::mutex mu;
    double *p = nullptr;
    size_t cap = 0, failed = 0;
    hipEvent_t ev = nullptr;
    hipStream_t last = nullptr;
    bool used = false;
    std::vector<hipEvent_t> pool;
    int event(size_t i)
    {
        if (pool.size() <= i) pool.resize(i + 1, nullptr);
        if (!pool[i]) SGPR_HIP(hipEventCreateWithFlags(&pool[i], hipEventDisableTiming));
        return 0;
    }
};
Scratch g_scratch[2][MAX_DEVICES];
bool lower_noscratch()
{
    static const bool forced_fail = tune("gemm_strassen_noscratch", 0) != 0;
    return forced_fail;
}
bool top_noscratch() { return tune("rec_strassen3_noscratch", 0) != 0; }

void scratch_free(Scratch &s)
{
    if (s.p) (void)hipFree(s.p);
    s.p = nullptr; s.cap = 0; s.used = false;
}
bool ensure(Scratch &s, size_t need, int sets, bool forced_fail)
{
    if (forced_fail) return false;
    if (s.cap >= need) return true;
    if (s.failed && need >= s.failed) return false;
    scratch_free(s);
    for (int b = sets; b >= 1; --b) {
        const size_t want = need * (size_t)b;
        if (s.failed && want >= s.failed) continue;
        if (hipMalloc((void **)&s.p, want * sizeof(double)) == hipSuccess) { s.cap = want; return true; }
        (void)hipGetLastError();
        s.p = nullptr;
        s.failed = want;
    }
    return false;
}
struct Use {
    Scratch &s; hipStream_t st; bool begun = false;
    Use(Scratch &s_, hipStream_t st_) : s(s_), st(st_) {}
    int begin()
    {
        if (!s.ev) SGPR_HIP(hipEventCreateWithFlags(&s.ev, hipEventDisableTiming));
        if (s.used && s.last != st) SGPR_HIP(hipStreamWaitEvent(st, s.ev, 0));
        begun = true;
        return 0;
    }
    ~Use()
    {
        if (!begun) return;
        if (hipEventRecord(s.ev, st) != hipSuccess) { (void)hipGetLastError(); (void)hipStreamSynchronize(st); }
        s.last = st;
        s.used = true;
    }
};

struct Join {
    hipStream_t st; int n; hipStream_t side[2]; hipEvent_t ev[2];
    ~Join()
    {
        for (int t = 0; t < n; ++t)
            if (hipEventRecord(ev[t], side[t]) != hipSuccess || hipStreamWaitEvent(st, ev[t], 0) != hipSuccess) {
                (void)hipGetLastError();
                (void)hipStreamSynchronize(side[t]);
            }
    }
};

int run_plan(const long long *recs, size_t nrec, double alpha, Mat A, Mat B, double beta, double *C, size_t ldc, double alpha2,
             double *C2, size_t ldc2, double *SA, double *SB, hipStream_t st, long sum_wgs = SUM_WGS)
{
    for (size_t i = 0; i < nrec; ++i) {
        const long long *r = recs + i * STRASSEN_REC;
        int rc = 0;
        if (r[0] == PLAN_SUM) {
            rc = sum_into(r, A, B, r[1] ? SB : SA, st, sum_wgs);
        } else if (r[0] == PLAN_PROD) {
            const int m = (int)r[7], n = (int)r[8], k = (int)r[9];
            const Mat X = operand_of(r, 0, A, SA), Y = operand_of(r, 1, B, SB);
            const Dests d = dests_of(r + 10, alpha, C, ldc);
            if (C2) {
                const Dests e = dests_of(r + 10, alpha2, C2, ldc2);
                double *cs[4] = {d.C1, nullptr, nullptr, nullptr};
                size_t ls[4] = {ldc, 0, 0, 0};
                double as[4] = {d.a1, 0.0, 0.0, 0.0};
                int cnt = 1;
                auto add = [&](double *p, size_t l, double a) { cs[cnt] = p; ls[cnt] = l; as[cnt] = a; ++cnt; };
                if (d.C2) add(d.C2, ldc, d.a2);
                add(e.C1, ldc2, e.a1);
                if (e.C2) add(e.C2, ldc2, e.a2);
                if (cnt == 2) rc = gemm_nt_two(m, n, k, as[0], X.p, X.ld, Y.p, Y.ld, 1.0, cs[0], ls[0], as[1], cs[1], ls[1], st);
                else          rc = gemm_nt_multi(m, n, k, X.p, X.ld, Y.p, Y.ld, 1.0, cnt, cs, ls, as, st);
            } else if (d.C2) {
                rc = gemm_nt_two(m, n, k, d.a1, X.p, X.ld, Y.p, Y.ld, 1.0, d.C1, ldc, d.a2, d.C2, ldc, st);
            } else {
                rc = gemm_nt(m, n, k, d.a1, X.p, X.ld, Y.p, Y.ld, 1.0, d.C1, ldc, 0, 0, st);
            }
        } else if (r[0] == PLAN_CLASSIC) {
            const double *Ap = block(A.p, A.ld, r[2], r[3]), *Bp = block(B.p, B.ld, r[4], r[5]);
            if (C2) rc = gemm_nt_two((int)r[6], (int)r[7], (int)r[8], alpha, Ap, A.ld, Bp, B.ld, beta, block(C, ldc, r[9], r[10]), ldc,
                                     alpha2, block(C2, ldc2, r[9], r[10]), ldc2, st);
            else    rc = gemm_nt((int)r[6], (int)r[7], (int)r[8], alpha, Ap, A.ld, Bp, B.ld, beta, block(C, ldc, r[9], r[10]), ldc, (int)r[1], 0, st);
        } else {
            set_error("run_plan: unknown record");
            rc = SGPR_E_ARG;
        }
        if (rc) return rc;
    }
    return 0;
}

int run_schedule(const std::vector<long long> &plan, const Plan2Cfg &c, const Need2 &nd, bool overlap, double alpha, Mat A, Mat B,
                 double beta, double *C, size_t ldc, Scratch &s, hipStream_t st)
{
    Use use(s, st);
    int rc = use.begin();
    if (rc) return rc;
    const SchedCfg sc = sched_cfg_of(nd, s.cap, overlap);
    std::vector<long long> sch;
    schedule_of(plan, c, nd, sc, sch);
    const size_t nrec = sch.size() / SCHED_REC;
    const long wgs = sc.nstreams ? side_wgs() : SUM_WGS;
    hipStream_t str[3] = {st, nullptr, nullptr};
    if (sc.nstreams && (rc = strassen_sum_streams(st, sc.nstreams, str + 1))) return rc;
    std::vector<char> needs(nrec, 0);
    for (size_t i = 0; i < nrec; ++i) {
        const long long *q = &sch[i * SCHED_REC];
        for (int j = 0; j < (int)q[20]; ++j)
            if (sch[(size_t)q[21 + j] * SCHED_REC + 17] != q[17]) needs[(size_t)q[21 + j]] = 1;
    }
    Join join{st, 0, {str[1], str[2]}, {nullptr, nullptr}};
    if (sc.nstreams) {
        if ((rc = s.event(0)) || (rc = s.event(1))) return rc;
        SGPR_HIP(hipEventRecord(s.pool[0], st));
        for (int t = 1; t <= sc.nstreams; ++t) SGPR_HIP(hipStreamWaitEvent(str[t], s.pool[0], 0));
        join.n = sc.nstreams; join.ev[0] = s.pool[0]; join.ev[1] = s.pool[1];
    }
    auto at = [&](int rg, long long b) { return s.p + sc.off[rg][b < 0 ? 0 : b]; };
    const long long *hd = nullptr;
    for (size_t i = 0; i < nrec; ++i) {
        const long long *q = &sch[i * SCHED_REC];
        hipStream_t me = str[q[17]];
        for (int j = 0; j < (int)q[20]; ++j) {
            const size_t w = (size_t)q[21 + j];
            if (sch[w * SCHED_REC + 17] != q[17]) SGPR_HIP(hipStreamWaitEvent(me, s.pool[2 + w], 0));
        }
        if (q[0] == PLAN2_PROD) {
            hd = q;
            continue;
        }
        double *const SA = at(0, q[0] == PLAN_SUM && q[1] ? 0 : q[18]), *const SB = at(1, q[0] == PLAN_SUM ? q[18] : q[19]);
        if (q[0] == PLAN2_SUM) {
            rc = sum_into(q, A, B, at(2 + (int)q[1], q[18]), me, wgs);
        } else if (q[16] == 0) {
            rc = run_plan(q, 1, alpha, A, B, beta, C, ldc, 0.0, nullptr, 0, SA, SB, me, wgs);
        } else {
            const Dests d = dests_of(hd + 10, alpha, C, ldc);
            rc = run_plan(q, 1, d.a1, operand_of(hd, 0, A, at(2, hd[18])), operand_of(hd, 1, B, at(3, hd[19])), 1.0, d.C1, ldc, d.a2, d.C2, ldc,
                          SA, SB, me, wgs);
        }
        if (rc) return rc;
        if (needs[i]) {
            if ((rc = s.event(2 + i))) return rc;
            SGPR_HIP(hipEventRecord(s.pool[2 + i], me));
        }
    }
    return 0;
}

int run_top(const std::vector<long long> &plan, const Need3 &nd, double alpha, Mat A, Mat B, double *C, size_t ldc, Scratch &s, hipStream_t st)
{
    Use use(s, st);
    int rc = use.begin();
    if (rc) return rc;
    const size_t need = nd.total();
    const bool overlap = tune("rec_strassen3_overlap", 1) != 0;
    const int nbuf = (top_buffers_wanted() >= 2 && s.cap >= 2 * need) ? 2 : 1;
    const long wgs = overlap ? side_wgs() : SUM_WGS;
    hipStream_t sd = st;
    if (overlap && (rc = strassen_top_stream(st, &sd))) return rc;
    auto at = [&](int region, int b) { return s.p + (size_t)b * need + (region == 0 ? 0 : (region == 1 ? nd.v[0] : nd.v[0] + nd.v[1])); };
    auto join = [&]() {
        if (!overlap) return 0;
        SGPR_HIP(hipEventRecord(s.pool[1], sd));
        SGPR_HIP(hipStreamWaitEvent(st, s.pool[1], 0));
        return 0;
    };
    if ((rc = s.event(0)) || (rc = s.event(1))) return rc;
    if (overlap) {
        SGPR_HIP(hipEventRecord(s.pool[0], st));
        SGPR_HIP(hipStreamWaitEvent(sd, s.pool[0], 0));
    }
    Join at_exit{st, overlap ? 1 : 0, {sd, nullptr}, {s.pool[1], nullptr}};
    struct Pend { const long long *r; int b; size_t p; };
    std::vector<Pend> pending;
    size_t p = 0;
    auto flush = [&]() {
        for (const Pend &q : pending) {
            if (overlap) SGPR_HIP(hipStreamWaitEvent(sd, s.pool[3 + 2 * q.p], 0));
            const Dests d = dests_of(q.r + 3, alpha, C, ldc);
            const int e = block_acc((int)q.r[1], (int)q.r[2], at(0, q.b), d.C1, d.a1, d.C2, d.a2, ldc, sd, wgs);
            if (e) return e;
        }
        pending.clear();
        return 0;
    };
    for (size_t i = 0; i + STRASSEN_REC <= plan.size(); i += STRASSEN_REC) {
        const long long *r = &plan[i];
        const int b = (int)(p % (size_t)nbuf);
        if (r[0] == PLAN3_SUM) {
            if (nbuf == 1 && (rc = flush())) return rc;
            rc = sum_into(r, A, B, at(1 + (int)r[1], b), sd, wgs);
        } else if (r[0] == PLAN3_ZERO) {
            if (nbuf == 1 && (rc = flush())) return rc;
            SGPR_HIP(hipMemsetAsync(at(0, b), 0, (size_t)r[1] * (size_t)r[2] * sizeof(double), sd));
        } else if (r[0] == PLAN3_PROD) {
            const int m = (int)r[7], n = (int)r[8], k = (int)r[9];
            if (overlap) {
                if ((rc = s.event(2 + 2 * p)) || (rc = s.event(3 + 2 * p))) return rc;
                SGPR_HIP(hipEventRecord(s.pool[2 + 2 * p], sd));
                SGPR_HIP(hipStreamWaitEvent(st, s.pool[2 + 2 * p], 0));
            }
            const Mat X = operand_of(r, 0, A, at(1, b)), Y = operand_of(r, 1, B, at(2, b));
            rc = gemm_nt_strassen_cfg(m, n, k, 1.0, X.p, X.ld, Y.p, Y.ld, 1.0, at(0, b), (size_t)m, 0, cfg_of_words(r + 10), st);
            if (rc) return rc;
            if (overlap) SGPR_HIP(hipEventRecord(s.pool[3 + 2 * p], st));
            rc = flush();
        } else if (r[0] == PLAN3_ACC) {
            pending.push_back(Pend{r, b, p});
            ++p;
        } else if (r[0] == PLAN3_PASS) {
            if ((rc = flush()) || (rc = join())) return rc;
            rc = gemm_nt_strassen_cfg((int)r[6], (int)r[7], (int)r[8], alpha, block(A.p, A.ld, r[2], r[3]), A.ld, block(B.p, B.ld, r[4], r[5]), B.ld,
                                      1.0, block(C, ldc, r[9], r[10]), ldc, (int)r[1], cfg_of_words(r + 11), st);
        } else {
            set_error("run_top: unknown record");
            rc = SGPR_E_ARG;
        }
        if (rc) return rc;
    }
    return flush();
}
}

void strassen_reserve(size_t both, size_t one, hipStream_t st)
{
    const int dev = device_of(st);
    if (dev < 0 || !strassen_levels()) return;
    Scratch &s = g_scratch[0][dev];
    std::lock_guard<std::mutex> lock(s.mu);
    if (both > one && !outer_noscratch() && ensure(s, both, 1, lower_noscratch())) return;
    if (one) (void)ensure(s, one, 1, lower_noscratch());
}
void strassen_top_reserve(size_t need, hipStream_t st)
{
    const int dev = device_of(st);
    if (dev < 0 || !need) return;
    Scratch &s = g_scratch[1][dev];
    std::lock_guard<std::mutex> lock(s.mu);
    if (s.cap >= need * (size_t)top_buffers_wanted()) return;
    if (s.cap >= need && s.failed && need * 2 >= s.failed) return;
    scratch_free(s);
    (void)ensure(s, need, top_buffers_wanted(), top_noscratch());
}
int strassen_trim()
{
    for (int level = 1; level >= 0; --level)
        for (Scratch &s : g_scratch[level]) {
            std::lock_guard<std::mutex> lock(s.mu);
            scratch_free(s);
            if (s.ev) (void)hipEventDestroy(s.ev);
            for (hipEvent_t e : s.pool) if (e) (void)hipEventDestroy(e);
            s.pool.clear();
            s.ev = nullptr; s.failed = 0; s.last = nullptr;
        }
    (void)hipGetLastError();
    return 0;
}

int gemm_nt_strassen(int m, int n, int k, double alpha, const double *A, size_t lda, const double *B, size_t ldb, double beta,
                     double *C, size_t ldc, int lower, hipStream_t st)
{
    return gemm_nt_strassen_cfg(m, n, k, alpha, A, lda, B, ldb, beta, C, ldc, lower, StrassenCfg{}, st);
}
int gemm_nt_strassen_rec(int m, int n, int k, double alpha, const double *A, size_t lda, const double *B, size_t ldb, double beta,
                         double *C, size_t ldc, int lower, hipStream_t st)
{
    return gemm_nt_strassen_cfg(m, n, k, alpha, A, lda, B, ldb, beta, C, ldc, lower, strassen_rec_cfg(strassen_rec_values(), k, lower), st);
}
int gemm_nt_strassen_cfg(int m, int n, int k, double alpha, const double *A, size_t lda, const double *B, size_t ldb, double beta,
                         double *C, size_t ldc, int lower, const StrassenCfg &cfg, hipStream_t st)
{
    const Plan2Cfg c2 = cfg2_of(cfg, ~(size_t)0);
    const bool aligned = ((((uintptr_t)A | (uintptr_t)B) & 15) == 0) && (((lda | ldb) & 1) == 0);
    if (std::min(m, n) / 2 < std::min(c2.in.smin, under_of(c2).smin) || !strassen_levels() || !aligned || beta != 1.0 || (lower && m != n))
        return gemm_nt(m, n, k, alpha, A, lda, B, ldb, beta, C, ldc, lower, 0, st);
    std::vector<long long> plan;
    int rc = 0;
    const int dev = device_of(st);
    const bool overlap = tune("gemm_strassen_overlap", 1) != 0;
    const Mat Am{A, lda}, Bm{B, ldb};
    if (strassen_levels() >= 2 && dev >= 0 && !outer_noscratch() && std::min(lower ? m / 2 : m, lower ? n / 2 : n) / 2 >= c2.smin2) {
        outer_plan_of(m, n, k, lower, c2, plan);
        const Need2 nd = plan_need(plan, c2);
        if (nd.v[2] + nd.v[3]) {
            Scratch &s = g_scratch[0][dev];
            std::lock_guard<std::mutex> lock(s.mu);
            if (ensure(s, nd.total(), 1, lower_noscratch())) return run_schedule(plan, c2, nd, overlap, alpha, Am, Bm, beta, C, ldc, s, st);
        }
    }
    auto unscratched = [&] { return run_plan(plan.data(), plan.size() / STRASSEN_REC, alpha, Am, Bm, beta, C, ldc, 0.0, nullptr, 0, nullptr, nullptr, st); };
    rc = strassen_plan(m, n, k, lower, c2.in.smin, c2.in.kslab, ~(size_t)0, plan);
    if (rc) return rc;
    Need2 nd = plan_need(plan, c2);
    if (!nd.total()) return unscratched();
    if (dev < 0) return gemm_nt(m, n, k, alpha, A, lda, B, ldb, beta, C, ldc, lower, 0, st);
    Scratch &s = g_scratch[0][dev];
    std::lock_guard<std::mutex> lock(s.mu);
    if (!ensure(s, nd.total(), 1, lower_noscratch())) {
        if ((rc = strassen_plan(m, n, k, lower, c2.in.smin, c2.in.kslab, s.cap, plan))) return rc;
        nd = plan_need(plan, c2);
        if (!nd.total()) return unscratched();
    }
    return run_schedule(plan, c2, nd, overlap, alpha, Am, Bm, beta, C, ldc, s, st);
}

int strassen_top_gemm(int m, int n, int k, double alpha, const double *A, size_t lda, const double *B, size_t ldb, double beta,
                      double *C, size_t ldc, int lower, const StrassenRec *vp, const StrassenTop *tp, hipStream_t st)
{
    const StrassenRec v = vp ? *vp : strassen_rec_values();
    const StrassenTop t = tp ? *tp : strassen_top_values();
    const StrassenCfg cfg = strassen_rec_cfg(v, k, lower);
    const bool aligned = ((((uintptr_t)A | (uintptr_t)B | (uintptr_t)C) & 15) == 0) && (((lda | ldb | ldc) & 1) == 0);
    const int dev = (!v.on || t.smin3 <= 0 || std::min(lower ? m / 2 : m, lower ? n / 2 : n) / 2 < t.smin3) ? -1 : device_of(st);
    if (dev < 0 || strassen_levels() < 2 || !aligned || beta != 1.0 || (lower && m != n))
        return gemm_nt_strassen_cfg(m, n, k, alpha, A, lda, B, ldb, beta, C, ldc, lower, cfg, st);
    std::vector<long long> plan;
    const int rc = strassen_top_plan(m, n, k, lower, &v, &t, ~(size_t)0, plan);
    if (rc) return rc;
    const Need3 nd = top_need(plan);
    if (nd.total()) {
        Scratch &s = g_scratch[1][dev];
        std::lock_guard<std::mutex> lock(s.mu);
        if (ensure(s, nd.total(), top_buffers_wanted(), top_noscratch())) return run_top(plan, nd, alpha, Mat{A, lda}, Mat{B, ldb}, C, ldc, s, st);
    }
    return gemm_nt_strassen_cfg(m, n, k, alpha, A, lda, B, ldb, beta, C, ldc, lower, cfg, st);
}

}
```

### sympgpr_amd/csrc/strassen_plan.hip

```cpp
#include <cstdlib>
#include <initializer_list>

#include "strassen.h"

namespace sgpr {
using namespace splan;

namespace {
void put(std::vector<long long> &out, std::initializer_list<long long> v)
{
    size_t i = 0;
    for (long long x : v) { out.push_back(x); ++i; }
    for (; i < STRASSEN_REC; ++i) out.push_back(0);
}
long slab_of(long k, const PlanCfg &c)
{
    if (k <= 0 || k % 32 != 0 || c.kslab < 32) return 0;
    const long nslab = (k + c.kslab - 1) / c.kslab;
    const long step = ((k + nslab - 1) / nslab + 31) / 32 * 32;
    const long kmin = std::max(c.smin / 2, 16L);
    const long last = k - (nslab - 1) * step;
    if (last <= 0 || step / 2 < kmin || last / 2 < kmin) return 0;
    return step;
}
bool qualifies(long m, long n, long k, const PlanCfg &c)
{
    if (m <= 0 || n <= 0 || m % 512 != 0 || n % 256 != 0) return false;
    if (m / 2 < c.smin || n / 2 < c.smin) return false;
    const long step = slab_of(k, c);
    if (!step) return false;
    return (size_t)(m / 2 + n / 2) * (size_t)(step / 2) <= c.scratch;
}
void seven(int kind_sum, int kind_prod, long m2, long n2, long k2, long k0, long ar, long br, long cr, long cc, std::vector<long long> &out)
{
    const long a1 = ar, a2 = ar + m2, b1 = br, b2 = br + n2, j1 = k0, j2 = k0 + k2;
    const long c1r = cr, c2r = cr + m2, c1c = cc, c2c = cc + n2;
    auto sum = [&](int side, long xr, long xc, long yr, long yc, int sign) {
        put(out, {kind_sum, side, side ? n2 : m2, k2, xr, xc, yr, yc, sign});
    };
    auto prod = [&](int as, long pr, long pc, int bs, long qr, long qc, long d1r, long d1c, int s1, long d2r, long d2c, int s2) {
        put(out, {kind_prod, as, pr, pc, bs, qr, qc, m2, n2, k2, d1r, d1c, s1, d2r, d2c, s2});
    };
    sum(0, a1, j1, a2, j2, +1); sum(1, b1, j1, b2, j2, +1);
    prod(1, 0, 0, 1, 0, 0, c1r, c1c, +1, c2r, c2c, +1);
    sum(0, a2, j1, a2, j2, +1);
    prod(1, 0, 0, 0, b1, j1, c2r, c1c, +1, c2r, c2c, -1);
    sum(1, b2, j1, b2, j2, -1);
    prod(0, a1, j1, 1, 0, 0, c1r, c2c, +1, c2r, c2c, +1);
    sum(1, b1, j2, b1, j1, -1);
    prod(0, a2, j2, 1, 0, 0, c1r, c1c, +1, c2r, c1c, +1);
    sum(0, a1, j1, a1, j2, +1);
    prod(1, 0, 0, 0, b2, j2, c1r, c1c, -1, c1r, c2c, +1);
    sum(0, a2, j1, a1, j1, -1); sum(1, b1, j1, b2, j1, +1);
    prod(1, 0, 0, 1, 0, 0, c2r, c2c, +1, 0, 0, 0);
    sum(0, a1, j2, a2, j2, -1); sum(1, b1, j2, b2, j2, +1);
    prod(1, 0, 0, 1, 0, 0, c1r, c1c, +1, 0, 0, 0);
}
void plan_gemm(long m, long n, long k, long ar, long br, long cr, long cc, const PlanCfg &c, std::vector<long long> &out)
{
    if (!qualifies(m, n, k, c)) { put(out, {PLAN_CLASSIC, 0, ar, 0, br, 0, m, n, k, cr, cc}); return; }
    const long step = slab_of(k, c);
    for (long k0 = 0; k0 < k; k0 += step) seven(PLAN_SUM, PLAN_PROD, m / 2, n / 2, std::min(step, k - k0) / 2, k0, ar, br, cr, cc, out);
}
void plan_syrk(long n, long k, long r0, const PlanCfg &c, std::vector<long long> &out)
{
    const long h = n / 2;
    if (n % 2 != 0 || !qualifies(h, h, k, c)) { put(out, {PLAN_CLASSIC, 1, r0, 0, r0, 0, n, n, k, r0, r0}); return; }
    plan_syrk(h, k, r0, c, out);
    plan_gemm(h, h, k, r0 + h, r0, r0 + h, r0, c, out);
    plan_syrk(h, k, r0 + h, c, out);
}
PlanCfg default_cfg()
{
    static const long smin = std::max(128L, (long)tune("gemm_strassen_min", 8192));
    static const long kslab = std::max(32L, (long)tune("gemm_strassen_kslab", 16384));
    return PlanCfg{smin, kslab, ~(size_t)0};
}
constexpr long REC_SMIN_GEMM = 4096, REC_SMIN_SYRK = 8192, REC_SMIN2_GEMM = 8192, REC_SMIN2_SYRK = 8192, REC_KSLAB2_SHORT = 16384;
constexpr long REC_SMIN3 = 16384, REC_KSLAB3 = 65536, REC_KSLAB3_SHORT = 32768;
Plan2Cfg default_cfg2()
{
    static const long smin2 = std::max(256L, (long)tune("gemm_strassen2_min", 16384));
    static const long kslab2 = std::max(64L, (long)tune("gemm_strassen2_kslab", 32768));
    return Plan2Cfg{default_cfg(), smin2, kslab2, ~(size_t)0};
}
bool qualifies2(long m, long n, long k, const Plan2Cfg &c)
{
    if (m <= 0 || n <= 0 || m % 1024 != 0 || n % 512 != 0) return false;
    if (m / 2 < c.smin2 || n / 2 < c.smin2) return false;
    if (c.kslab2 < 64 || c.kslab2 % 64 != 0 || k < c.kslab2) return false;
    const size_t pair = (size_t)(m / 2 + n / 2) * (size_t)(c.kslab2 / 2);
    if (pair > c.scratch) return false;
    PlanCfg ci = under_of(c);
    ci.scratch = c.scratch - pair;
    return qualifies(m / 2, n / 2, c.kslab2 / 2, ci);
}
PlanCfg inner_of(const Plan2Cfg &c) { return PlanCfg{c.in.smin, c.in.kslab, c.scratch}; }
void plan2_gemm(long m, long n, long k, long ar, long br, long cr, long cc, const Plan2Cfg &c, std::vector<long long> &out)
{
    if (!qualifies2(m, n, k, c)) { plan_gemm(m, n, k, ar, br, cr, cc, inner_of(c), out); return; }
    long k0 = 0;
    for (; k0 + c.kslab2 <= k; k0 += c.kslab2) seven(PLAN2_SUM, PLAN2_PROD, m / 2, n / 2, c.kslab2 / 2, k0, ar, br, cr, cc, out);
    if (k0 == k) return;
    size_t i = out.size();
    plan_gemm(m, n, k - k0, ar, br, cr, cc, inner_of(c), out);
    for (; i + STRASSEN_REC <= out.size(); i += STRASSEN_REC) {
        long long *r = &out[i];
        if (r[0] == PLAN_SUM) { r[5] += k0; r[7] += k0; }
        else if (r[0] == PLAN_PROD) { if (!r[1]) r[3] += k0; if (!r[4]) r[6] += k0; }
        else { r[3] += k0; r[5] += k0; }
    }
}
void plan2_syrk(long n, long k, long r0, const Plan2Cfg &c, std::vector<long long> &out)
{
    const long h = n / 2;
    if (n % 2 != 0 || !qualifies2(h, h, k, c)) { plan_syrk(n, k, r0, inner_of(c), out); return; }
    plan2_syrk(h, k, r0, c, out);
    plan2_gemm(h, h, k, r0 + h, r0, r0 + h, r0, c, out);
    plan2_syrk(h, k, r0 + h, c, out);
}
void inner_plan(const long long *r, const PlanCfg &ci, std::vector<long long> &out)
{
    out.clear();
    plan_gemm(r[7], r[8], r[9], 0, 0, 0, 0, ci, out);
}
}

int splan::strassen_levels()
{
    static const int lv = [] { const char *e = getenv("SGPR_GEMM_STRASSEN"); return !e ? 2 : (e[0] == '0' ? 0 : (e[0] == '1' ? 1 : 2)); }();
    return lv;
}
bool splan::outer_noscratch()
{
    static const bool forced_fail = tune("gemm_strassen2_noscratch", 0) != 0;
    return forced_fail;
}
PlanCfg splan::under_of(const Plan2Cfg &c) { return PlanCfg{c.smin_under >= 0 ? c.smin_under : c.in.smin, c.in.kslab, c.in.scratch}; }
Plan2Cfg splan::cfg2_of(const StrassenCfg &cfg, size_t scratch_doubles)
{
    Plan2Cfg c = default_cfg2();
    if (cfg.smin >= 0) c.in.smin = std::max(128L, cfg.smin);
    if (cfg.kslab >= 0) c.in.kslab = std::max(32L, cfg.kslab);
    if (cfg.smin2 >= 0) c.smin2 = std::max(256L, cfg.smin2);
    if (cfg.kslab2 >= 0) c.kslab2 = std::max(64L, cfg.kslab2);
    if (cfg.smin_under >= 0) c.smin_under = std::max(128L, cfg.smin_under);
    c.scratch = scratch_doubles;
    return c;
}
void splan::outer_plan_of(int m, int n, int k, int lower, const Plan2Cfg &c, std::vector<long long> &out)
{
    out.clear();
    if (lower) plan2_syrk(n, k, 0, c, out);
    else       plan2_gemm(m, n, k, 0, 0, 0, 0, c, out);
}
Need2 splan::plan_need(const std::vector<long long> &plan, const Plan2Cfg &c)
{
    Need2 nd;
    std::vector<long long> in;
    auto sums = [&](const long long *r, int base) {
        size_t &v = nd.v[base + r[1]];
        v = std::max(v, (size_t)r[2] * (size_t)r[3]);
    };
    PlanCfg ci = under_of(c);
    ci.scratch = ~(size_t)0;
    for (size_t i = 0; i + STRASSEN_REC <= plan.size(); i += STRASSEN_REC) {
        const long long *r = &plan[i];
        if (r[0] == PLAN_SUM) sums(r, 0);
        else if (r[0] == PLAN2_SUM) sums(r, 2);
        else if (r[0] == PLAN2_PROD) {
            inner_plan(r, ci, in);
            for (size_t j = 0; j + STRASSEN_REC <= in.size(); j += STRASSEN_REC)
                if (in[j] == PLAN_SUM) sums(&in[j], 0);
        }
    }
    return nd;
}

SchedCfg splan::sched_cfg_of(const Need2 &nd, size_t cap, bool overlap)
{
    SchedCfg sc;
    size_t pos = 0;
    for (int r = 0; r < 4; ++r) { sc.off[r][0] = pos; pos += nd.v[r]; }
    sc.nstreams = !overlap ? 0 : (tune("gemm_strassen_overlap_streams", 1) >= 2 ? 2 : 1);
    if (!overlap) return sc;
    const double lim = tune("gemm_strassen_overlap_slack", -1);
    size_t slack = cap > nd.total() ? cap - nd.total() : 0;
    if (lim >= 0) slack = std::min(slack, (size_t)lim);
    for (int r = 0; r < 4; ++r) {
        if (!nd.v[r]) continue;
        if (nd.v[r] > slack) break;
        sc.nbuf[r] = 2; sc.off[r][1] = pos; pos += nd.v[r]; slack -= nd.v[r];
    }
    return sc;
}
void splan::schedule_of(const std::vector<long long> &plan, const Plan2Cfg &c, const Need2 &nd, const SchedCfg &sc, std::vector<long long> &out)
{
    struct Buf { long long writer = -1, prod_reader = -1, sum_reader[2] = {-1, -1}; };
    Buf buf[4][2];
    int next[4] = {0, 0, 0, 0}, cur[4] = {0, 0, 0, 0};
    out.clear();
    auto emit = [&](const long long *r, int level) {
        const size_t at = out.size();
        out.resize(at + SCHED_REC, 0);
        for (int j = 0; j < STRASSEN_REC; ++j) out[at + j] = r[j];
        out[at + 16] = level; out[at + 18] = out[at + 19] = -1;
        return at;
    };
    auto wait = [&](size_t at, long long idx) {
        if (idx < 0) return;
        const int nw = (int)out[at + 20];
        for (int j = 0; j < nw; ++j) if (out[at + 21 + j] == idx) return;
        if (nw < SCHED_REC - 21) { out[at + 21 + nw] = idx; out[at + 20] = nw + 1; }
    };
    auto read = [&](size_t at, int rg, int b) {
        wait(at, buf[rg][b].writer);
        buf[rg][b].prod_reader = (long long)(at / SCHED_REC);
    };
    auto sum = [&](const long long *r, int level, int rg, int src, int sb) {
        const size_t at = emit(r, level);
        const long long idx = (long long)(at / SCHED_REC);
        const int stream = sc.nstreams == 2 ? 1 + (int)r[1] : std::min(sc.nstreams, 1), b = next[rg];
        next[rg] = (b + 1) % sc.nbuf[rg];
        Buf &t = buf[rg][b];
        wait(at, t.prod_reader); wait(at, t.sum_reader[0]); wait(at, t.sum_reader[1]);
        if (!out[at + 20]) wait(at, t.writer);
        if (src >= 0) { wait(at, buf[src][sb].writer); buf[src][sb].sum_reader[std::max(stream - 1, 0)] = idx; }
        t = Buf{};
        t.writer = idx;
        cur[rg] = b;
        out[at + 17] = stream; out[at + 18] = b;
    };
    PlanCfg ci = under_of(c);
    ci.scratch = nd.inner();
    std::vector<long long> in;
    for (size_t i = 0; i + STRASSEN_REC <= plan.size(); i += STRASSEN_REC) {
        const long long *r = &plan[i];
        if (r[0] == PLAN_SUM || r[0] == PLAN2_SUM) {
            sum(r, 0, (r[0] == PLAN2_SUM ? 2 : 0) + (int)r[1], -1, 0);
        } else if (r[0] == PLAN_PROD) {
            const size_t at = emit(r, 0);
            if (r[1]) { out[at + 18] = cur[0]; read(at, 0, cur[0]); }
            if (r[4]) { out[at + 19] = cur[1]; read(at, 1, cur[1]); }
        } else if (r[0] == PLAN2_PROD) {
            const size_t hd = emit(r, 0);
            const int xa = r[1] ? cur[2] : -1, yb = r[4] ? cur[3] : -1;
            out[hd + 18] = xa; out[hd + 19] = yb;
            inner_plan(r, ci, in);
            for (size_t j = 0; j + STRASSEN_REC <= in.size(); j += STRASSEN_REC) {
                const long long *q = &in[j];
                if (q[0] == PLAN_SUM) {
                    const int ob = q[1] ? yb : xa;
                    sum(q, 1, (int)q[1], ob >= 0 ? 2 + (int)q[1] : -1, std::max(ob, 0));
                    continue;
                }
                const size_t at = emit(q, 1);
                const bool a_scr = q[0] == PLAN_PROD && q[1], b_scr = q[0] == PLAN_PROD && q[4];
                if (a_scr) { out[at + 18] = cur[0]; read(at, 0, cur[0]); } else if (xa >= 0) read(at, 2, xa);
                if (b_scr) { out[at + 19] = cur[1]; read(at, 1, cur[1]); } else if (yb >= 0) read(at, 3, yb);
            }
        } else {
            (void)emit(r, 0);
        }
    }
}

int strassen_plan(int m, int n, int k, int lower, long smin, long kslab, size_t scratch_doubles, std::vector<long long> &out)
{
    if (bad_extents(m, n, k, lower)) { set_error("strassen_plan: bad extents"); return SGPR_E_ARG; }
    PlanCfg c = default_cfg();
    if (smin >= 0) c.smin = std::max(128L, smin);
    if (kslab >= 0) c.kslab = std::max(32L, kslab);
    c.scratch = scratch_doubles;
    out.clear();
    if (lower) plan_syrk(n, k, 0, c, out);
    else       plan_gemm(m, n, k, 0, 0, 0, 0, c, out);
    return 0;
}
int strassen_outer_plan(int m, int n, int k, int lower, long smin, long kslab, long smin2, long kslab2, size_t scratch_doubles,
                   std::vector<long long> &out)
{
    if (bad_extents(m, n, k, lower)) { set_error("strassen_outer_plan: bad extents"); return SGPR_E_ARG; }
    outer_plan_of(m, n, k, lower, cfg2_of(StrassenCfg{smin, kslab, smin2, kslab2, -1}, scratch_doubles), out);
    return 0;
}

StrassenRec strassen_rec_values()
{
    StrassenRec v;
    v.on = getenv("SGPR_GEMM_STRASSEN") == nullptr;
    const Plan2Cfg lib = default_cfg2();
    v.smin_gemm = std::max(128L, (long)tune("rec_strassen_min_gemm", std::min(REC_SMIN_GEMM, lib.in.smin)));
    v.smin_syrk = std::max(128L, (long)tune("rec_strassen_min_syrk", std::min(REC_SMIN_SYRK, lib.in.smin)));
    v.smin2_gemm = std::max(256L, (long)tune("rec_strassen2_min_gemm", std::min(REC_SMIN2_GEMM, lib.smin2)));
    v.smin2_syrk = std::max(256L, (long)tune("rec_strassen2_min_syrk", std::min(REC_SMIN2_SYRK, lib.smin2)));
    v.kslab = std::max(32L, (long)tune("rec_strassen_kslab", lib.in.kslab));
    v.kslab2 = std::max(64L, (long)tune("rec_strassen2_kslab", lib.kslab2));
    v.kslab2_short = (long)tune("rec_strassen2_kslab_short", REC_KSLAB2_SHORT);
    if (v.kslab2_short < 64 || v.kslab2_short % 64 != 0 || v.kslab2_short >= v.kslab2) v.kslab2_short = 0;
    return v;
}
StrassenCfg strassen_rec_cfg(const StrassenRec &v, int k, int lower)
{
    StrassenCfg c;
    if (!v.on) return c;
    c.smin = lower ? v.smin_syrk : v.smin_gemm;
    c.smin2 = lower ? v.smin2_syrk : v.smin2_gemm;
    c.smin_under = std::min(c.smin, c.smin2 / 2);
    c.kslab = v.kslab;
    c.kslab2 = (k < v.kslab2 && v.kslab2_short > 0 && k >= v.kslab2_short) ? v.kslab2_short : v.kslab2;
    return c;
}
int strassen_rec_plan(int m, int n, int k, int lower, long cfg_out[5], size_t scratch_doubles, std::vector<long long> &out)
{
    if (bad_extents(m, n, k, lower)) { set_error("strassen_rec_plan: bad extents"); return SGPR_E_ARG; }
    const Plan2Cfg c = cfg2_of(strassen_rec_cfg(strassen_rec_values(), k, lower), scratch_doubles);
    if (cfg_out) cfg_to_words(StrassenCfg{c.in.smin, c.in.kslab, c.smin2, c.kslab2, under_of(c).smin}, cfg_out);
    outer_plan_of(m, n, k, lower, c, out);
    return 0;
}

int strassen_schedule(int m, int n, int k, int lower, long long cap_doubles, long long info[12], std::vector<long long> &out)
{
    if (bad_extents(m, n, k, lower)) { set_error("strassen_schedule: bad extents"); return SGPR_E_ARG; }
    const Plan2Cfg c = cfg2_of(strassen_rec_cfg(strassen_rec_values(), k, lower), ~(size_t)0);
    std::vector<long long> plan;
    if (strassen_levels() >= 2 && !outer_noscratch()) outer_plan_of(m, n, k, lower, c, plan);
    else {
        const int rc = strassen_plan(m, n, k, lower, c.in.smin, c.in.kslab, ~(size_t)0, plan);
        if (rc) return rc;
    }
    const Need2 nd = plan_need(plan, c);
    const size_t cap = cap_doubles < 0 ? nd.total() : (size_t)cap_doubles;
    if (cap < nd.total()) { set_error("strassen_schedule: the capacity is below the call's need"); return SGPR_E_ARG; }
    const SchedCfg sc = sched_cfg_of(nd, cap, true);
    schedule_of(plan, c, nd, sc, out);
    if (info) {
        for (int i = 0; i < 12; ++i) info[i] = 0;
        for (int r = 0; r < 4; ++r) { info[r] = (long long)nd.v[r]; info[4 + r] = sc.nbuf[r]; }
        info[8] = sc.nstreams; info[9] = (long long)cap;
    }
    return 0;
}

size_t strassen_scratch_doubles_cfg(int m, int n, int k, int lower, int levels, const StrassenCfg &cfg)
{
    std::vector<long long> plan;
    if (!strassen_levels() || bad_extents(m, n, k, lower)) return 0;
    const Plan2Cfg c2 = cfg2_of(cfg, ~(size_t)0);
    if (levels >= 2 && strassen_levels() >= 2) outer_plan_of(m, n, k, lower, c2, plan);
    else if (strassen_plan(m, n, k, lower, c2.in.smin, c2.in.kslab, ~(size_t)0, plan)) return 0;
    return plan_need(plan, c2).total();
}

namespace {
long top_slab(long k, const StrassenTop &t)
{
    const long s = (t.kslab3 > 0 && k >= t.kslab3) ? t.kslab3 : t.kslab3_short;
    return (s >= 128 && s % 128 == 0 && k >= s) ? s : 0;
}
bool top_qualifies(long m, long n, long k, const StrassenRec &v, const StrassenTop &t, size_t scratch)
{
    if (!v.on || t.smin3 <= 0 || m <= 0 || n <= 0 || m % 2048 != 0 || n % 1024 != 0) return false;
    if (m / 2 < t.smin3 || n / 2 < t.smin3) return false;
    const long slab = top_slab(k, t);
    return slab && (size_t)(m / 2) * (size_t)(n / 2) + (size_t)(m / 2 + n / 2) * (size_t)(slab / 2) <= scratch;
}
void put_cfg(std::vector<long long> &out, int at, const StrassenCfg &c) { cfg_to_words(c, &out[out.size() - STRASSEN_REC + at]); }
void top_pass(int lower, long ar, long ac, long br, long bc, long m, long n, long k, long cr, long cc, int kind, const StrassenRec &v,
              std::vector<long long> &out)
{
    put(out, {PLAN3_PASS, lower, ar, ac, br, bc, m, n, k, cr, cc});
    put_cfg(out, 11, strassen_rec_cfg(v, (int)k, kind));
}
void top_gemm(long m, long n, long k, long ar, long br, long cr, long cc, int kind, const StrassenRec &v, const StrassenTop &t,
              size_t scratch, std::vector<long long> &out)
{
    if (!top_qualifies(m, n, k, v, t, scratch)) { top_pass(0, ar, 0, br, 0, m, n, k, cr, cc, kind, v, out); return; }
    const long slab = top_slab(k, t), m2 = m / 2, n2 = n / 2, k2 = slab / 2;
    std::vector<long long> seven_recs;
    long k0 = 0;
    for (; k0 + slab <= k; k0 += slab) {
        seven_recs.clear();
        seven(PLAN3_SUM, PLAN3_PROD, m2, n2, k2, k0, ar, br, cr, cc, seven_recs);
        for (size_t i = 0; i + STRASSEN_REC <= seven_recs.size(); i += STRASSEN_REC) {
            const long long *r = &seven_recs[i];
            if (r[0] == PLAN3_SUM) { out.insert(out.end(), r, r + STRASSEN_REC); continue; }
            put(out, {PLAN3_ZERO, m2, n2});
            put(out, {PLAN3_PROD, r[1], r[2], r[3], r[4], r[5], r[6], r[7], r[8], r[9]});
            put_cfg(out, 10, strassen_rec_cfg(v, (int)k2, kind));
            put(out, {PLAN3_ACC, m2, n2, r[10], r[11], r[12], r[13], r[14], r[15]});
        }
    }
    if (k0 < k) top_pass(0, ar, k0, br, k0, m, n, k - k0, cr, cc, kind, v, out);
}
void top_syrk(long n, long k, const StrassenRec &v, const StrassenTop &t, size_t scratch, std::vector<long long> &out)
{
    const long h = n / 2;
    if (n % 2 != 0 || !top_qualifies(h, h, k, v, t, scratch)) { top_pass(1, 0, 0, 0, 0, n, n, k, 0, 0, 1, v, out); return; }
    top_pass(1, 0, 0, 0, 0, h, h, k, 0, 0, 1, v, out);
    top_gemm(h, h, k, h, 0, h, 0, 1, v, t, scratch, out);
    top_pass(1, h, 0, h, 0, h, h, k, h, h, 1, v, out);
}
}

Need3 splan::top_need(const std::vector<long long> &plan)
{
    Need3 nd;
    for (size_t i = 0; i + STRASSEN_REC <= plan.size(); i += STRASSEN_REC) {
        const long long *r = &plan[i];
        if (r[0] == PLAN3_ZERO) nd.v[0] = std::max(nd.v[0], (size_t)r[1] * (size_t)r[2]);
        else if (r[0] == PLAN3_SUM) nd.v[1 + r[1]] = std::max(nd.v[1 + r[1]], (size_t)r[2] * (size_t)r[3]);
    }
    return nd;
}
int splan::top_buffers_wanted() { return (tune("rec_strassen3_overlap", 1) != 0 && tune("rec_strassen3_buffers", 2) >= 2) ? 2 : 1; }

StrassenTop strassen_top_values()
{
    StrassenTop t;
    t.smin3 = std::max(0L, (long)tune("rec_strassen3_min", (double)REC_SMIN3));
    t.kslab3 = std::max(0L, (long)tune("rec_strassen3_kslab", (double)REC_KSLAB3));
    t.kslab3_short = std::max(0L, (long)tune("rec_strassen3_kslab_short", (double)REC_KSLAB3_SHORT));
    return t;
}
int strassen_top_plan(int m, int n, int k, int lower, const StrassenRec *vp, const StrassenTop *tp, size_t scratch_doubles,
                      std::vector<long long> &out)
{
    const StrassenRec v = vp ? *vp : strassen_rec_values();
    const StrassenTop t = tp ? *tp : strassen_top_values();
    if (bad_extents(m, n, k, lower)) { set_error("strassen_top_plan: bad extents"); return SGPR_E_ARG; }
    out.clear();
    if (lower) top_syrk(n, k, v, t, scratch_doubles, out);
    else       top_gemm(m, n, k, 0, 0, 0, 0, 0, v, t, scratch_doubles, out);
    return 0;
}
int strassen_cfg_plan(int m, int n, int k, int lower, const long cfg[5], std::vector<long long> &out)
{
    if (bad_extents(m, n, k, lower) || !cfg) { set_error("strassen_cfg_plan: bad arguments"); return SGPR_E_ARG; }
    outer_plan_of(m, n, k, lower, cfg2_of(cfg_of_words(cfg), ~(size_t)0), out);
    return 0;
}
size_t strassen_top_scratch_doubles(int m, int n, int k, int lower, const StrassenRec &v, const StrassenTop &t)
{
    std::vector<long long> plan;
    if (strassen_levels() < 2 || strassen_top_plan(m, n, k, lower, &v, &t, ~(size_t)0, plan)) return 0;
    return top_need(plan).total();
}

}
```

Before: 84.59.

## Chain Strassen schedules across consecutive GEMM calls to overlap side-stream sums

Carries scratch-buffer ownership and per-slot events from one Strassen GEMM schedule into the next call on the same stream. The following call's side streams then wait only on the buffers they reuse instead of a full entry join. In run_top, PASS GEMMs skip the join when their output does not overlap unjoined accumulations, and the first sum uses full workgroups. The block accumulate kernel also processes two columns per step instead of four to cut register pressure. The risk is more event bookkeeping and subtle cross-call hazards if the carry state is wrong.

After: 84.83 (median of 6 runs). About the same (+0.3%).

```diff
diff --git a/include/sympgpr_probe.h b/include/sympgpr_probe.h
--- a/include/sympgpr_probe.h
+++ b/include/sympgpr_probe.h
@@ -45,6 +45,9 @@
                                      double beta, double *C, size_t ldc, int lower, void *stream);
 int sgpr_probe_strassen_schedule(int m, int n, int k, int lower, long capacity_doubles, long long info[12], long long *out,
                                  int max_records, int *count);
+int sgpr_probe_strassen_chain_schedule(int ncalls, const long long *calls, long long *info, long long *out, int max_records, int *count);
+int sgpr_probe_strassen_chain_counts(unsigned long long out[2]);
+int sgpr_probe_block_acc_dev(int rows, int cols, const double *T, double *C1, double a1, double *C2, double a2, size_t ldc, void *stream);
 int sgpr_probe_batch_layout(int path, int mode, int d, int reg, int nbatch, int n_pts, int nhyp, unsigned long long out[24]);
 int sgpr_probe_batch_layout_nd_loo(int path, int mode, int d, int nbatch, int n_pts, int nhyp, unsigned long long out[24]);
 int sgpr_probe_batch_layout_loograd_mid(int d, int reg, int nbatch, int n_pts, int nhyp, unsigned long long out[32]);
diff --git a/sympgpr_amd/_lib.py b/sympgpr_amd/_lib.py
--- a/sympgpr_amd/_lib.py
+++ b/sympgpr_amd/_lib.py
@@ -207,6 +207,11 @@
     "sgpr_probe_strassen_rec_scratch": (C.c_int, [C.c_int, C.POINTER(C.c_ulonglong)]),
     "sgpr_probe_strassen_schedule": (C.c_int, [C.c_int, C.c_int, C.c_int, C.c_int, C.c_long, C.POINTER(C.c_longlong),
                                                C.POINTER(C.c_longlong), C.c_int, C.POINTER(C.c_int)]),
+    "sgpr_probe_strassen_chain_schedule": (C.c_int, [C.c_int, C.POINTER(C.c_longlong), C.POINTER(C.c_longlong), C.POINTER(C.c_longlong),
+                                                     C.c_int, C.POINTER(C.c_int)]),
+    "sgpr_probe_strassen_chain_counts": (C.c_int, [C.POINTER(C.c_ulonglong)]),
+    "sgpr_probe_block_acc_dev": (C.c_int, [C.c_int, C.c_int, C.c_void_p, C.c_void_p, C.c_double, C.c_void_p, C.c_double, C.c_size_t,
+                                           C.c_void_p]),
     "sgpr_probe_gemm_strassen_rec_dev": (C.c_int, [C.c_int, C.c_int, C.c_int, C.c_double, C.c_void_p, C.c_size_t, C.c_void_p, C.c_size_t,
                                                    C.c_double, C.c_void_p, C.c_size_t, C.c_int, C.c_void_p]),
     "sgpr_probe_strassen_top_plan": (C.c_int, [C.c_int, C.c_int, C.c_int, C.c_int, C.c_long, C.POINTER(C.c_longlong), C.c_int,
diff --git a/sympgpr_amd/csrc/probe.hip b/sympgpr_amd/csrc/probe.hip
--- a/sympgpr_amd/csrc/probe.hip
+++ b/sympgpr_amd/csrc/probe.hip
@@ -566,6 +566,28 @@
     for (size_t i = 0; out && i < sched.size() && (int)(i / SCHED_REC) < max_records; ++i) out[i] = sched[i];
     return 0;
 }
+extern "C" int sgpr_probe_strassen_chain_schedule(int ncalls, const long long *calls, long long *info, long long *out, int max_records,
+                                                  int *count)
+{
+    if (!count) { set_error("probe_strassen_chain_schedule: bad arguments"); return SGPR_E_ARG; }
+    std::vector<long long> sched;
+    const int rc = strassen_chain_schedule(ncalls, calls, info, sched);
+    if (rc) return rc;
+    *count = (int)(sched.size() / SCHED_REC);
+    for (size_t i = 0; out && i < sched.size() && (int)(i / SCHED_REC) < max_records; ++i) out[i] = sched[i];
+    return 0;
+}
+extern "C" int sgpr_probe_strassen_chain_counts(unsigned long long out[2])
+{
+    if (!out) { set_error("probe_strassen_chain_counts: bad arguments"); return SGPR_E_ARG; }
+    strassen_chain_counts(out);
+    return 0;
+}
+extern "C" int sgpr_probe_block_acc_dev(int rows, int cols, const double *T, double *C1, double a1, double *C2, double a2, size_t ldc,
+                                        void *stream)
+{
+    return strassen_block_acc(rows, cols, T, C1, a1, C2, a2, ldc, static_cast<hipStream_t>(stream));
+}
 extern "C" int sgpr_probe_gemm_strassen_rec_dev(int m, int n, int k, double alpha, const double *A, size_t lda, const double *B, size_t ldb,
                                                 double beta, double *C, size_t ldc, int lower, void *stream)
 {
diff --git a/sympgpr_amd/csrc/strassen.h b/sympgpr_amd/csrc/strassen.h
--- a/sympgpr_amd/csrc/strassen.h
+++ b/sympgpr_amd/csrc/strassen.h
@@ -37,6 +37,8 @@
 int strassen_rec_plan(int m, int n, int k, int lower, long cfg_out[5], size_t scratch_doubles, std::vector<long long> &out);
 
 constexpr int SCHED_REC = 32;
+constexpr int SCHED_CARRY_WAIT = 26, SCHED_CARRY_RECORD = 27;
+int strassen_chain_schedule(int ncalls, const long long *calls, long long *info, std::vector<long long> &out);
 int strassen_schedule(int m, int n, int k, int lower, long long cap_doubles, long long info[12], std::vector<long long> &out);
 
 enum { PLAN3_SUM = 6, PLAN3_ZERO = 7, PLAN3_PROD = 8, PLAN3_ACC = 9, PLAN3_PASS = 10 };
@@ -69,6 +71,19 @@
     size_t off[4][2] = {};
     int nstreams = 1;
 };
+struct Carry {
+    bool valid = false;
+    SchedCfg sc;
+    int next[4] = {0, 0, 0, 0};
+    bool have[4][2] = {};
+    bool fits(const SchedCfg &o) const
+    {
+        if (!valid || o.nstreams < 1 || o.nstreams != sc.nstreams) return false;
+        for (int r = 0; r < 4; ++r)
+            if (o.nbuf[r] != sc.nbuf[r] || o.off[r][0] != sc.off[r][0] || o.off[r][1] != sc.off[r][1]) return false;
+        return true;
+    }
+};
 struct Need3 { size_t v[3] = {0, 0, 0}; size_t total() const { return v[0] + v[1] + v[2]; } };
 
 int strassen_levels();
@@ -78,7 +93,8 @@
 void outer_plan_of(int m, int n, int k, int lower, const Plan2Cfg &c, std::vector<long long> &out);
 Need2 plan_need(const std::vector<long long> &plan, const Plan2Cfg &c);
 SchedCfg sched_cfg_of(const Need2 &nd, size_t cap, bool overlap);
-void schedule_of(const std::vector<long long> &plan, const Plan2Cfg &c, const Need2 &nd, const SchedCfg &sc, std::vector<long long> &out);
+void schedule_of(const std::vector<long long> &plan, const Plan2Cfg &c, const Need2 &nd, const SchedCfg &sc, std::vector<long long> &out,
+                 Carry *carry = nullptr, bool *chained = nullptr);
 Need3 top_need(const std::vector<long long> &plan);
 int top_buffers_wanted();
 }
@@ -92,6 +108,8 @@
                          double *C, size_t ldc, int lower, hipStream_t st);
 int strassen_top_gemm(int m, int n, int k, double alpha, const double *A, size_t lda, const double *B, size_t ldb, double beta,
                       double *C, size_t ldc, int lower, const StrassenRec *v, const StrassenTop *t, hipStream_t st);
+int strassen_block_acc(int rows, int cols, const double *T, double *C1, double a1, double *C2, double a2, size_t ldc, hipStream_t st);
+void strassen_chain_counts(unsigned long long out[2]);
 void strassen_reserve(size_t both, size_t one, hipStream_t st);
 void strassen_top_reserve(size_t need, hipStream_t st);
 int strassen_trim();
diff --git a/sympgpr_amd/csrc/strassen.hip b/sympgpr_amd/csrc/strassen.hip
--- a/sympgpr_amd/csrc/strassen.hip
+++ b/sympgpr_amd/csrc/strassen.hip
@@ -1,4 +1,5 @@
 #include <algorithm>
+#include <atomic>
 #include <cstdint>
 #include <mutex>
 #include <vector>
@@ -46,20 +47,23 @@
         const int cg = (int)(p / nrc), rc = (int)(p - (long)cg * nrc);
         const int r = rc * 512 + 2 * (int)threadIdx.x;
         if (r >= rows) continue;
-        double2_t t[4], c1[4], c2[4];
+#pragma unroll 1
+        for (int c0 = cg * 4; c0 < min(cg * 4 + 4, cols); c0 += 2) {
+            double2_t t[2], c1[2], c2[2];
 #pragma unroll
-        for (int u = 0; u < 4; ++u) {
-            const int c = min(cg * 4 + u, cols - 1);
-            t[u] = *reinterpret_cast<const double2_t *>(T + (size_t)r + (size_t)c * (size_t)rows);
-            c1[u] = *reinterpret_cast<const double2_t *>(C1 + (size_t)r + (size_t)c * ldc);
-            if (C2) c2[u] = *reinterpret_cast<const double2_t *>(C2 + (size_t)r + (size_t)c * ldc);
-        }
+            for (int u = 0; u < 2; ++u) {
+                const int c = min(c0 + u, cols - 1);
+                t[u] = *reinterpret_cast<const double2_t *>(T + (size_t)r + (size_t)c * (size_t)rows);
+                c1[u] = *reinterpret_cast<const double2_t *>(C1 + (size_t)r + (size_t)c * ldc);
+                if (C2) c2[u] = *reinterpret_cast<const double2_t *>(C2 + (size_t)r + (size_t)c * ldc);
+            }
 #pragma unroll
-        for (int u = 0; u < 4; ++u) {
-            const int c = cg * 4 + u;
-            if (c >= cols) continue;
-            *reinterpret_cast<double2_t *>(C1 + (size_t)r + (size_t)c * ldc) = c1[u] + a1 * t[u];
-            if (C2) *reinterpret_cast<double2_t *>(C2 + (size_t)r + (size_t)c * ldc) = c2[u] + a2 * t[u];
+            for (int u = 0; u < 2; ++u) {
+                const int c = c0 + u;
+                if (c >= cols) continue;
+                *reinterpret_cast<double2_t *>(C1 + (size_t)r + (size_t)c * ldc) = c1[u] + a1 * t[u];
+                if (C2) *reinterpret_cast<double2_t *>(C2 + (size_t)r + (size_t)c * ldc) = c2[u] + a2 * t[u];
+            }
         }
     }
 }
@@ -109,6 +113,13 @@
     hipStream_t last = nullptr;
     bool used = false;
     std::vector<hipEvent_t> pool;
+    Carry carry;
+    hipEvent_t cev[8] = {};
+    int carried(int slot)
+    {
+        if (!cev[slot]) SGPR_HIP(hipEventCreateWithFlags(&cev[slot], hipEventDisableTiming));
+        return 0;
+    }
     int event(size_t i)
     {
         if (pool.size() <= i) pool.resize(i + 1, nullptr);
@@ -117,6 +128,7 @@
     }
 };
 Scratch g_scratch[2][MAX_DEVICES];
+std::atomic<unsigned long long> g_chain_counts[2];
 bool lower_noscratch()
 {
     static const bool forced_fail = tune("gemm_strassen_noscratch", 0) != 0;
@@ -128,6 +140,7 @@
 {
     if (s.p) (void)hipFree(s.p);
     s.p = nullptr; s.cap = 0; s.used = false;
+    s.carry = Carry{};
 }
 bool ensure(Scratch &s, size_t need, int sets, bool forced_fail)
 {
@@ -219,17 +232,24 @@
     return 0;
 }
 
+struct Entry { hipEvent_t ready; };
 int run_schedule(const std::vector<long long> &plan, const Plan2Cfg &c, const Need2 &nd, bool overlap, double alpha, Mat A, Mat B,
-                 double beta, double *C, size_t ldc, Scratch &s, hipStream_t st)
-{
+                 double beta, double *C, size_t ldc, Scratch &s, hipStream_t st, const Entry *entry)
+{
+    const bool same_user = s.used && s.last == st;
     Use use(s, st);
     int rc = use.begin();
     if (rc) return rc;
     const SchedCfg sc = sched_cfg_of(nd, s.cap, overlap);
+    const bool chain_on = sc.nstreams && tune("rec_strassen3_chain", 1) != 0;
+    Carry carry = (chain_on && entry && same_user) ? s.carry : Carry{};
+    s.carry = Carry{};
+    bool chained = false;
     std::vector<long long> sch;
-    schedule_of(plan, c, nd, sc, sch);
+    schedule_of(plan, c, nd, sc, sch, chain_on && entry ? &carry : nullptr, &chained);
+    if (chain_on && entry) ++g_chain_counts[chained ? 0 : 1];
     const size_t nrec = sch.size() / SCHED_REC;
-    const long wgs = sc.nstreams ? side_wgs() : SUM_WGS;
+    const long side = sc.nstreams ? side_wgs() : SUM_WGS;
     hipStream_t str[3] = {st, nullptr, nullptr};
     if (sc.nstreams && (rc = strassen_sum_streams(st, sc.nstreams, str + 1))) return rc;
     std::vector<char> needs(nrec, 0);
@@ -241,12 +261,13 @@
     Join join{st, 0, {str[1], str[2]}, {nullptr, nullptr}};
     if (sc.nstreams) {
         if ((rc = s.event(0)) || (rc = s.event(1))) return rc;
-        SGPR_HIP(hipEventRecord(s.pool[0], st));
-        for (int t = 1; t <= sc.nstreams; ++t) SGPR_HIP(hipStreamWaitEvent(str[t], s.pool[0], 0));
+        if (!chained) SGPR_HIP(hipEventRecord(s.pool[0], st));
+        for (int t = 1; t <= sc.nstreams; ++t) SGPR_HIP(hipStreamWaitEvent(str[t], chained ? entry->ready : s.pool[0], 0));
         join.n = sc.nstreams; join.ev[0] = s.pool[0]; join.ev[1] = s.pool[1];
     }
     auto at = [&](int rg, long long b) { return s.p + sc.off[rg][b < 0 ? 0 : b]; };
     const long long *hd = nullptr;
+    bool alone = chain_on && !chained;
     for (size_t i = 0; i < nrec; ++i) {
         const long long *q = &sch[i * SCHED_REC];
         hipStream_t me = str[q[17]];
@@ -254,10 +275,14 @@
             const size_t w = (size_t)q[21 + j];
             if (sch[w * SCHED_REC + 17] != q[17]) SGPR_HIP(hipStreamWaitEvent(me, s.pool[2 + w], 0));
         }
+        if (q[SCHED_CARRY_WAIT]) SGPR_HIP(hipStreamWaitEvent(me, s.cev[q[SCHED_CARRY_WAIT] - 1], 0));
         if (q[0] == PLAN2_PROD) {
             hd = q;
             continue;
         }
+        const bool is_sum = q[0] == PLAN_SUM || q[0] == PLAN2_SUM;
+        const long wgs = is_sum && alone ? SUM_WGS : side;
+        alone = alone && is_sum;
         double *const SA = at(0, q[0] == PLAN_SUM && q[1] ? 0 : q[18]), *const SB = at(1, q[0] == PLAN_SUM ? q[18] : q[19]);
         if (q[0] == PLAN2_SUM) {
             rc = sum_into(q, A, B, at(2 + (int)q[1], q[18]), me, wgs);
@@ -273,9 +298,18 @@
             if ((rc = s.event(2 + i))) return rc;
             SGPR_HIP(hipEventRecord(s.pool[2 + i], me));
         }
-    }
+        for (int slot = 0; slot < 8; ++slot)
+            if (q[SCHED_CARRY_RECORD] >> slot & 1) {
+                if ((rc = s.carried(slot))) return rc;
+                SGPR_HIP(hipEventRecord(s.cev[slot], me));
+            }
+    }
+    s.carry = carry;
     return 0;
 }
+
+int front_end(int m, int n, int k, double alpha, const double *A, size_t lda, const double *B, size_t ldb, double beta, double *C, size_t ldc,
+              int lower, const StrassenCfg &cfg, hipStream_t st, const Entry *entry);
 
 int run_top(const std::vector<long long> &plan, const Need3 &nd, double alpha, Mat A, Mat B, double *C, size_t ldc, Scratch &s, hipStream_t st)
 {
@@ -285,15 +319,24 @@
     const size_t need = nd.total();
     const bool overlap = tune("rec_strassen3_overlap", 1) != 0;
     const int nbuf = (top_buffers_wanted() >= 2 && s.cap >= 2 * need) ? 2 : 1;
+    const bool chain = overlap && tune("rec_strassen3_chain", 1) != 0;
     const long wgs = overlap ? side_wgs() : SUM_WGS;
     hipStream_t sd = st;
     if (overlap && (rc = strassen_top_stream(st, &sd))) return rc;
     auto at = [&](int region, int b) { return s.p + (size_t)b * need + (region == 0 ? 0 : (region == 1 ? nd.v[0] : nd.v[0] + nd.v[1])); };
+    struct Rect { long long r, c, rows, cols; };
+    std::vector<Rect> unjoined;
     auto join = [&]() {
+        unjoined.clear();
         if (!overlap) return 0;
         SGPR_HIP(hipEventRecord(s.pool[1], sd));
         SGPR_HIP(hipStreamWaitEvent(st, s.pool[1], 0));
         return 0;
+    };
+    auto touches_unjoined = [&](const Rect &x) {
+        for (const Rect &y : unjoined)
+            if (x.r < y.r + y.rows && y.r < x.r + x.rows && x.c < y.c + y.cols && y.c < x.c + x.cols) return true;
+        return false;
     };
     if ((rc = s.event(0)) || (rc = s.event(1))) return rc;
     if (overlap) {
@@ -308,6 +351,8 @@
         for (const Pend &q : pending) {
             if (overlap) SGPR_HIP(hipStreamWaitEvent(sd, s.pool[3 + 2 * q.p], 0));
             const Dests d = dests_of(q.r + 3, alpha, C, ldc);
+            unjoined.push_back(Rect{q.r[3], q.r[4], q.r[1], q.r[2]});
+            if (q.r[8]) unjoined.push_back(Rect{q.r[6], q.r[7], q.r[1], q.r[2]});
             const int e = block_acc((int)q.r[1], (int)q.r[2], at(0, q.b), d.C1, d.a1, d.C2, d.a2, ldc, sd, wgs);
             if (e) return e;
         }
@@ -319,7 +364,7 @@
         const int b = (int)(p % (size_t)nbuf);
         if (r[0] == PLAN3_SUM) {
             if (nbuf == 1 && (rc = flush())) return rc;
-            rc = sum_into(r, A, B, at(1 + (int)r[1], b), sd, wgs);
+            rc = sum_into(r, A, B, at(1 + (int)r[1], b), sd, chain && p == 0 ? SUM_WGS : wgs);
         } else if (r[0] == PLAN3_ZERO) {
             if (nbuf == 1 && (rc = flush())) return rc;
             SGPR_HIP(hipMemsetAsync(at(0, b), 0, (size_t)r[1] * (size_t)r[2] * sizeof(double), sd));
@@ -331,7 +376,8 @@
                 SGPR_HIP(hipStreamWaitEvent(st, s.pool[2 + 2 * p], 0));
             }
             const Mat X = operand_of(r, 0, A, at(1, b)), Y = operand_of(r, 1, B, at(2, b));
-            rc = gemm_nt_strassen_cfg(m, n, k, 1.0, X.p, X.ld, Y.p, Y.ld, 1.0, at(0, b), (size_t)m, 0, cfg_of_words(r + 10), st);
+            const Entry behind_zero{overlap ? s.pool[2 + 2 * p] : nullptr};
+            rc = front_end(m, n, k, 1.0, X.p, X.ld, Y.p, Y.ld, 1.0, at(0, b), (size_t)m, 0, cfg_of_words(r + 10), st, chain ? &behind_zero : nullptr);
             if (rc) return rc;
             if (overlap) SGPR_HIP(hipEventRecord(s.pool[3 + 2 * p], st));
             rc = flush();
@@ -339,9 +385,11 @@
             pending.push_back(Pend{r, b, p});
             ++p;
         } else if (r[0] == PLAN3_PASS) {
-            if ((rc = flush()) || (rc = join())) return rc;
-            rc = gemm_nt_strassen_cfg((int)r[6], (int)r[7], (int)r[8], alpha, block(A.p, A.ld, r[2], r[3]), A.ld, block(B.p, B.ld, r[4], r[5]), B.ld,
-                                      1.0, block(C, ldc, r[9], r[10]), ldc, (int)r[1], cfg_of_words(r + 11), st);
+            if ((rc = flush())) return rc;
+            if ((!chain || touches_unjoined(Rect{r[9], r[10], r[6], r[7]})) && (rc = join())) return rc;
+            const Entry at_entry{s.pool[0]};
+            rc = front_end((int)r[6], (int)r[7], (int)r[8], alpha, block(A.p, A.ld, r[2], r[3]), A.ld, block(B.p, B.ld, r[4], r[5]), B.ld, 1.0,
+                           block(C, ldc, r[9], r[10]), ldc, (int)r[1], cfg_of_words(r + 11), st, chain ? &at_entry : nullptr);
         } else {
             set_error("run_top: unknown record");
             rc = SGPR_E_ARG;
@@ -352,6 +400,19 @@
 }
 }
 
+void strassen_chain_counts(unsigned long long out[2])
+{
+    out[0] = g_chain_counts[0].load();
+    out[1] = g_chain_counts[1].load();
+}
+int strassen_block_acc(int rows, int cols, const double *T, double *C1, double a1, double *C2, double a2, size_t ldc, hipStream_t st)
+{
+    if (rows <= 0 || cols <= 0 || rows % 2 || ldc % 2 || ldc < (size_t)rows || !T || !C1 || (((uintptr_t)T | (uintptr_t)C1 | (uintptr_t)C2) & 15)) {
+        set_error("strassen_block_acc: bad arguments");
+        return SGPR_E_ARG;
+    }
+    return block_acc(rows, cols, T, C1, a1, C2, a2, ldc, st, side_wgs());
+}
 void strassen_reserve(size_t both, size_t one, hipStream_t st)
 {
     const int dev = device_of(st);
@@ -381,6 +442,7 @@
             if (s.ev) (void)hipEventDestroy(s.ev);
             for (hipEvent_t e : s.pool) if (e) (void)hipEventDestroy(e);
             s.pool.clear();
+            for (hipEvent_t &e : s.cev) { if (e) (void)hipEventDestroy(e); e = nullptr; }
             s.ev = nullptr; s.failed = 0; s.last = nullptr;
         }
     (void)hipGetLastError();
@@ -399,6 +461,12 @@
 }
 int gemm_nt_strassen_cfg(int m, int n, int k, double alpha, const double *A, size_t lda, const double *B, size_t ldb, double beta,
                          double *C, size_t ldc, int lower, const StrassenCfg &cfg, hipStream_t st)
+{
+    return front_end(m, n, k, alpha, A, lda, B, ldb, beta, C, ldc, lower, cfg, st, nullptr);
+}
+namespace {
+int front_end(int m, int n, int k, double alpha, const double *A, size_t lda, const double *B, size_t ldb, double beta, double *C, size_t ldc,
+              int lower, const StrassenCfg &cfg, hipStream_t st, const Entry *entry)
 {
     const Plan2Cfg c2 = cfg2_of(cfg, ~(size_t)0);
     const bool aligned = ((((uintptr_t)A | (uintptr_t)B) & 15) == 0) && (((lda | ldb) & 1) == 0);
@@ -415,7 +483,7 @@
         if (nd.v[2] + nd.v[3]) {
             Scratch &s = g_scratch[0][dev];
             std::lock_guard<std::mutex> lock(s.mu);
-            if (ensure(s, nd.total(), 1, lower_noscratch())) return run_schedule(plan, c2, nd, overlap, alpha, Am, Bm, beta, C, ldc, s, st);
+            if (ensure(s, nd.total(), 1, lower_noscratch())) return run_schedule(plan, c2, nd, overlap, alpha, Am, Bm, beta, C, ldc, s, st, entry);
         }
     }
     auto unscratched = [&] { return run_plan(plan.data(), plan.size() / STRASSEN_REC, alpha, Am, Bm, beta, C, ldc, 0.0, nullptr, 0, nullptr, nullptr, st); };
@@ -431,7 +499,8 @@
         nd = plan_need(plan, c2);
         if (!nd.total()) return unscratched();
     }
-    return run_schedule(plan, c2, nd, overlap, alpha, Am, Bm, beta, C, ldc, s, st);
+    return run_schedule(plan, c2, nd, overlap, alpha, Am, Bm, beta, C, ldc, s, st, entry);
+}
 }
 
 int strassen_top_gemm(int m, int n, int k, double alpha, const double *A, size_t lda, const double *B, size_t ldb, double beta,
diff --git a/sympgpr_amd/csrc/strassen_plan.hip b/sympgpr_amd/csrc/strassen_plan.hip
--- a/sympgpr_amd/csrc/strassen_plan.hip
+++ b/sympgpr_amd/csrc/strassen_plan.hip
@@ -194,11 +194,18 @@
     }
     return sc;
 }
-void splan::schedule_of(const std::vector<long long> &plan, const Plan2Cfg &c, const Need2 &nd, const SchedCfg &sc, std::vector<long long> &out)
+void splan::schedule_of(const std::vector<long long> &plan, const Plan2Cfg &c, const Need2 &nd, const SchedCfg &sc, std::vector<long long> &out,
+                        Carry *carry, bool *chained)
 {
     struct Buf { long long writer = -1, prod_reader = -1, sum_reader[2] = {-1, -1}; };
     Buf buf[4][2];
     int next[4] = {0, 0, 0, 0}, cur[4] = {0, 0, 0, 0};
+    const bool chain = carry && carry->fits(sc);
+    long long last[4][2] = {{-1, -1}, {-1, -1}, {-1, -1}, {-1, -1}};
+    bool written[4][2] = {};
+    if (chained) *chained = chain;
+    if (carry && !chain) *carry = Carry{};
+    if (chain) for (int r = 0; r < 4; ++r) next[r] = carry->next[r] % sc.nbuf[r];
     out.clear();
     auto emit = [&](const long long *r, int level) {
         const size_t at = out.size();
@@ -215,7 +222,7 @@
     };
     auto read = [&](size_t at, int rg, int b) {
         wait(at, buf[rg][b].writer);
-        buf[rg][b].prod_reader = (long long)(at / SCHED_REC);
+        buf[rg][b].prod_reader = last[rg][b] = (long long)(at / SCHED_REC);
     };
     auto sum = [&](const long long *r, int level, int rg, int src, int sb) {
         const size_t at = emit(r, level);
@@ -230,6 +237,11 @@
         t.writer = idx;
         cur[rg] = b;
         out[at + 17] = stream; out[at + 18] = b;
+        if (carry && !written[rg][b]) {
+            written[rg][b] = true;
+            if (chain && carry->have[rg][b]) out[at + SCHED_CARRY_WAIT] = 1 + 2 * rg + b;
+            carry->have[rg][b] = false;
+        }
     };
     PlanCfg ci = under_of(c);
     ci.scratch = nd.inner();
@@ -263,6 +275,16 @@
             (void)emit(r, 0);
         }
     }
+    if (!carry) return;
+    for (int rg = 0; rg < 4; ++rg)
+        for (int b = 0; b < 2; ++b)
+            if (last[rg][b] >= 0) {
+                out[(size_t)last[rg][b] * SCHED_REC + SCHED_CARRY_RECORD] |= 1LL << (2 * rg + b);
+                carry->have[rg][b] = true;
+            }
+    for (int r = 0; r < 4; ++r) carry->next[r] = next[r];
+    carry->sc = sc;
+    carry->valid = sc.nstreams >= 1;
 }
 
 int strassen_plan(int m, int n, int k, int lower, long smin, long kslab, size_t scratch_doubles, std::vector<long long> &out)
@@ -339,6 +361,45 @@
         for (int i = 0; i < 12; ++i) info[i] = 0;
         for (int r = 0; r < 4; ++r) { info[r] = (long long)nd.v[r]; info[4 + r] = sc.nbuf[r]; }
         info[8] = sc.nstreams; info[9] = (long long)cap;
+    }
+    return 0;
+}
+
+int strassen_chain_schedule(int ncalls, const long long *calls, long long *info, std::vector<long long> &out)
+{
+    if (ncalls < 0 || (ncalls && (!calls || !info))) { set_error("strassen_chain_schedule: bad arguments"); return SGPR_E_ARG; }
+    out.clear();
+    long long need = 0;
+    std::vector<std::vector<long long>> plans((size_t)ncalls);
+    std::vector<Plan2Cfg> cfgs;
+    for (int i = 0; i < ncalls; ++i) {
+        const long long *a = calls + 5 * i;
+        if (bad_extents((int)a[0], (int)a[1], (int)a[2], (int)a[3])) { set_error("strassen_chain_schedule: bad extents"); return SGPR_E_ARG; }
+        cfgs.push_back(cfg2_of(strassen_rec_cfg(strassen_rec_values(), (int)a[2], (int)a[3]), ~(size_t)0));
+        if (strassen_levels() >= 2 && !outer_noscratch()) outer_plan_of((int)a[0], (int)a[1], (int)a[2], (int)a[3], cfgs[i], plans[i]);
+        else {
+            const int rc = strassen_plan((int)a[0], (int)a[1], (int)a[2], (int)a[3], cfgs[i].in.smin, cfgs[i].in.kslab, ~(size_t)0, plans[i]);
+            if (rc) return rc;
+        }
+        need = std::max(need, (long long)plan_need(plans[i], cfgs[i]).total());
+    }
+    Carry carry;
+    long long cap_before = -1;
+    std::vector<long long> sch;
+    for (int i = 0; i < ncalls; ++i) {
+        const Need2 nd = plan_need(plans[i], cfgs[i]);
+        const long long cap = calls[5 * i + 4] < 0 ? need : calls[5 * i + 4];
+        if ((size_t)cap < nd.total()) { set_error("strassen_chain_schedule: the capacity is below the call's need"); return SGPR_E_ARG; }
+        if (cap != cap_before) carry = Carry{};
+        cap_before = cap;
+        const SchedCfg sc = sched_cfg_of(nd, (size_t)cap, true);
+        bool chained = false;
+        schedule_of(plans[i], cfgs[i], nd, sc, sch, &carry, &chained);
+        out.insert(out.end(), sch.begin(), sch.end());
+        long long *f = info + 12 * i;
+        for (int j = 0; j < 12; ++j) f[j] = 0;
+        for (int r = 0; r < 4; ++r) { f[r] = (long long)nd.v[r]; f[4 + r] = sc.nbuf[r]; }
+        f[8] = sc.nstreams; f[9] = cap; f[10] = chained; f[11] = (long long)(sch.size() / SCHED_REC);
     }
     return 0;
 }
```
